# LANL-Bioinformatics/PCRamp

Measured on AMD Instinct MI355X. Metric: primer-pair x target amplification evals/sec, higher is better.
Workload: dtype u32

## Files before the change

### pcramp_amd/csrc/pcr_device.hip

```cpp
#include <hip/hip_runtime.h>
#include <cstring>
#include <rocprim/device/device_radix_sort.hpp>

#include <stdint.h>
#include <string.h>
#include <math.h>
#include <stdlib.h>
#include <string>
#include <vector>
#include <chrono>
#include <algorithm>
#include <unordered_map>
#include <type_traits>
#include <thread>
#include <mutex>
#include <condition_variable>
#include <functional>
#include <memory>
#include <atomic>
#include <cassert>
#include <sched.h>
#include <pthread.h>

#include "../../include/pcramp_hip.h"
// ... 464 lines not shown
		for(uint32_t j = k >> 1;j > 0;j >>= 1){
			for(uint32_t i = tid;i < np2;i += FINBIG_THREADS){
				const uint32_t l = i ^ j;
				if(l > i){
					const uint64_t a = fin_keys[i], b = fin_keys[l];
					const bool up = ((i & k) == 0);
					if((a > b) == up){ fin_keys[i] = b; fin_keys[l] = a; }
				}
			}
			__syncthreads();
		}
	}
	const uint32_t chunk = (np2 + FINBIG_THREADS - 1)/FINBIG_THREADS;
	const uint32_t lo = min(np2, tid*chunk), hi = min(np2, lo + chunk);
	uint32_t cnt = 0;
	for(uint32_t i = lo;i < hi;++i){
		const uint64_t k = fin_keys[i];
		if(k != ~0ull && (i == 0 || fin_keys[i - 1] != k)) ++cnt;
	}
	part[tid] = cnt;
	__syncthreads();
	if(tid == 0){
		uint32_t run = 0;
		for(int t = 0;t < FINBIG_THREADS;++t){ const uint32_t c = part[t]; part[t] = run; run += c; }
		seg_hi[seq] = seq*cap + run;
	}
	__syncthreads();
	uint32_t rank = part[tid];
	for(uint32_t i = lo;i < hi;++i){
		const uint64_t k = fin_keys[i];
		if(k != ~0ull && (i == 0 || fin_keys[i - 1] != k)){
			DevEntry e;
			materialise_entry(k, planes, blk_off, irr, irr_off, e);
			db[(size_t)seq*cap + rank] = e;
			++rank;
		}
	}
}

#include "pcr_screen.inc"

#include "pcr_sw.inc"
#include "pcr_thermo.inc"

constexpr uint32_t N_TOUCHED_UNKNOWN = 0xFFFFFFFFu;
constexpr uint32_t EPOCH_LIMIT = (1u << 24) - 1;

struct SeqSet {
	uint32_t n = 0;
	std::vector<std::vector<uint8_t> > packed;
	std::vector<uint64_t> len, blk_off, nblk_real;
	std::vector<float> weight; DevBuf<float> d_weight; bool weight_dirty = true;
	std::vector<uint8_t> active;
	std::vector<std::vector<pcrhost::IrrEntry> > irr_host;
	uint64_t total_blocks = 0;
	uint32_t n_tiles = 0, n_irr = 0;
	bool ctrl_clean = false;
	bool touched_from_seg = false;
	uint32_t bucket_cap = 64;
	DevBuf<uint32_t> irr_perm; uint32_t irr_size_count[256];
	DevBuf<uint4> planes;
	DevBuf<uint32_t> valid, nib, tb, blk_seq, tile_seq, tile_pos0, irr_off, degen_tiles;
	uint32_t *valid_d() const { return valid.p + S2_VALID_FRONT; }
	uint32_t *tb_d() const { return tb.p + S2_TB_FRONT; }
	DevBuf<uint8_t> tile_degen; uint32_t n_degen_tiles = 0;
	DevBuf<TileDesc> tile_desc;
	DevBuf<uint64_t> d_len, d_blk_off, d_nblk_real;
	DevBuf<uint8_t> d_active;
	std::vector<uint8_t> has_eos; DevBuf<uint8_t> d_has_eos;
	DevBuf<IrrDev> irr;
	DevBuf<IrrScan> irr_scan;
	DevBuf<uint32_t> irx_first, irx_last, irx_words, irx_sums; bool irx_valid = false, irx_usable = false;
	uint32_t irr_n_multi = 0;
	DevBuf<uint32_t> pix_first, pix_last, pix_sums, blk_info, blk_local, blk_tile0; DevBuf<uint4> pix_ent; std::vector<uint32_t> pix_start_h; uint64_t pix_generation = 0; bool pix_valid = false, pix_usable = false;
	DevBuf<uint8_t> codes; DevBuf<uint64_t> d_code_off; bool have_codes = false;
	bool have_db = false;
	uint32_t n_entries = 0;
	uint32_t db_cap = 0;
	uint64_t n_slots = 0;
	DevBuf<DevEntry> db;
	DevBuf<uint32_t> touched;
	DevBuf<uint32_t> ctrl;
	uint32_t n_touched = 0;
	bool touched_built = false;
	uint32_t *d_seg_hi = nullptr;
};

}

struct HostPool {
	std::vector<std::thread> th;
	std::mutex m; std::condition_variable cv_go, cv_done;
	std::function<void(unsigned)> fn; unsigned n_parts = 0, next = 0, pending = 0; uint64_t gen = 0; bool stop = false;
	explicit HostPool(unsigned n_workers){ for(unsigned i = 0;i < n_workers;++i) th.emplace_back([this]{ work(); }); }
	~HostPool(){ { std::lock_guard<std::mutex> lk(m); stop = true; } cv_go.notify_all(); for(std::thread &t : th) t.join(); }
	unsigned size() const { return (unsigned)th.size(); }
	void work()
	{
		uint64_t seen = 0;
		std::unique_lock<std::mutex> lk(m);
		while(true){
			cv_go.wait(lk, [&]{ return stop || gen != seen; });
			if(stop) return;
			seen = gen;
			while(next < n_parts){ const unsigned p = next++; lk.unlock(); fn(p); lk.lock(); }
			if(--pending == 0) cv_done.notify_one();
		}
	}
	void run(unsigned parts, std::function<void(unsigned)> f)
	{
		std::unique_lock<std::mutex> lk(m);
		fn = std::move(f); n_parts = parts; next = 0; pending = (unsigned)th.size(); ++gen;
		cv_go.notify_all();
		while(next < n_parts){ const unsigned p = next++; lk.unlock(); fn(p); lk.lock(); }
		cv_done.wait(lk, [&]{ return pending == 0; });
	}
};

namespace { struct PassJob; struct Launcher; }

struct ItemBufs {
	DevBuf<uint8_t> *tmp; DevBuf<uint32_t> *cnt; DevBuf<uint64_t> *eoff; DevBuf<uint2> *items;
	DevBuf<uint64_t> *joff; DevBuf<float4> *res; DevBuf<uint2> *item_tm; DevBuf<uint32_t> *flag;
};
struct ItemScratch {
	DevBuf<uint8_t> in, tmp; DevBuf<uint32_t> cnt, flag; DevBuf<uint64_t> eoff, joff, ioff; DevBuf<uint2> items, item_tm; DevBuf<float4> res;
	ItemBufs bufs() { return ItemBufs{&tmp, &cnt, &eoff, &items, &joff, &res, &item_tm, &flag}; }
};

struct pcr_ctx {
	int device = 0;
	std::unique_ptr<HostPool> pool_;
	HostPool &host_pool()
	{
		if(!pool_){ const unsigned hw = std::max(1u, std::thread::hardware_concurrency()); pool_.reset(new HostPool(std::min(hw, 16u) - 1u)); }
		return *pool_;
	}
	Stream stream;
	Stream aux_stream;
	std::string design_text;
	DevBuf<uint64_t> split_where;
	pcr_params params;
	pcrhost::PackFilter filt;
	SeqSet sets[PCR_N_SETS];
	DevBuf<uint32_t> best, counters, mask, status;
	int scan_version = 3;
	bool force_seed1 = false;
	pcrseed::Lister seed_lists;
	static constexpr int S3_CHUNK_SETS = pcrseed::CHUNK_SETS;
	struct S2Key { uint32_t a, c, g, t, floor_; bool operator==(const S2Key &o) const { return a == o.a && c == o.c && g == o.g && t == o.t && floor_ == o.floor_; } };
	struct S2KeyHash { size_t operator()(const S2Key &k) const { uint64_t h = 0x9E3779B97F4A7C15ull; for(uint32_t v : {k.a, k.c, k.g, k.t, k.floor_}){ h ^= v; h *= 0x100000001B3ull; h ^= h >> 29; } return (size_t)h; } };
	struct S2Entry { std::vector<uint32_t> seeds;  uint32_t off_mask; bool seedable; };
	std::vector<pcrhost::Seed> s2_tmp;
	struct S3Launch { Seed3Slices W; uint32_t n_chunks, per_wg, slice_cap, n_irr_wg; };
	int pair_mode = 1; bool s3_pair_attr_set = false;
	bool no_seed3 = false, s3_attr_set = false;
	bool s3_next = true;
	bool s2_attr_set = false; uint32_t s2_dbg = 0; bool no_irr_index = false;
	std::unordered_map<S2Key, S2Entry, S2KeyHash> s1_cache;
	DevBuf<uint32_t> s1_image, s1_heads, s1_multi, s1_part;
	bool host_seed_tables = false;
	DevBuf<Hit> hits;
	DevBuf<uint64_t> bits_fr, bits_rf;
	DevBuf<OligoDev> oligos;
	DevBuf<SwJob> sw_jobs; DevBuf<SwOut> sw_out; DevBuf<uint8_t> sw_q, sw_qlen, sw_t, entry_codes, entry_lens;
	DevBuf<AmpRec> amp_recs, amp_recs2; DevBuf<BgPairDev> bg_pairs;
	DevBuf<uint64_t> amp_keys; DevBuf<uint32_t> amp_pkeys, amp_pair_start; DevBuf<uint8_t> sort_tmp;
	DevBuf<thermo::Job> th_jobs; DevBuf<thermo::JobOut> th_out; DevBuf<int> th_dg; DevBuf<uint2> th_map; DevBuf<uint32_t> th_bad;
	float th_dg_salt = -1.0f;
	DevBuf<unsigned long long> th_dbg; bool th_attr_set = false;
	std::vector<thermo::Job> th_host_jobs; std::vector<thermo::JobOut> th_host_res;
	MappedBuf<uint8_t> sw_pin; Event sw_done[2];
	DevBuf<pcr_amplicon> mx_amp;
	DevBuf<OligoDev> opt_oligos; DevBuf<uint2> opt_jobs; DevBuf<float> opt_cov; DevBuf<uint32_t> opt_loc, opt_tasks;
	DevBuf<Planes> mx_keys; uint32_t mx_n_keys = 0; DevBuf<uint32_t> mx_count;
	DevBuf<uint8_t> pool_in, pool_tmp; DevBuf<uint32_t> pool_cnt, pool_ord; DevBuf<uint64_t> pool_eoff, pool_ioff, pool_keys; DevBuf<uint2> pool_items; DevBuf<pcr_product> pool_rec;
	DevBuf<uint8_t> site_in, site_tmp; DevBuf<uint32_t> site_cnt, site_ord, site_flag; DevBuf<uint64_t> site_eoff, site_joff, site_keys; DevBuf<uint2> site_items; DevBuf<float4> site_res; DevBuf<pcr_site> site_rec;
	bool site_attr_set = false;
	DevBuf<uint8_t> sv_item; DevBuf<uint32_t> sv_ord, sv_var, sv_start, sv_vord, sv_map; DevBuf<pcr_site_variant> sv_rec; DevBuf<uint64_t> sv_vkeys;
	bool sv_attr_set = false;
	DevBuf<uint4> rp_foot; DevBuf<uint64_t> rp_keys; DevBuf<uint32_t> rp_u32; DevBuf<uint8_t> rp_state; DevBuf<pcr_repair_step> rp_rec;
	pcr_comm *shard_comm = nullptr; uint64_t shard_first = 0, shard_n_total = 0; int shard_mode = 0;
	DevBuf<uint64_t> sh_rec, sh_full; DevBuf<uint8_t> sh_stage;
	std::vector<uint64_t> shard_bounds; DevBuf<uint64_t> d_shard_bounds;
	bool design_ready = false; DevBuf<uint64_t> sh_bits;
	std::vector<std::vector<uint8_t> > samp_packed; std::vector<uint64_t> samp_len;
	void drop_shard(){ shard_comm = nullptr; shard_mode = 0; shard_bounds.clear(); design_ready = false; samp_packed.clear(); samp_len.clear(); }
	pcr_comm *trial_comm = nullptr;
	size_t amp_cap = size_t(1) << 20;
	uint32_t n_cu = 256;
	DevBuf<uint64_t> fin_scratch;
	std::vector<uint16_t> seed_count; std::vector<uint8_t> seed_fill, seed_own;
	uint32_t epoch = 0;
	uint32_t debug_epoch = 0;
	bool opt_pm_global = false;
	uint32_t opt_dbg_wg_tasks = 0, opt_dbg_task_cap = 0;
	uint64_t best_seen = 0;
	static constexpr int STAGE_RING = 4;
	struct StageSlot { MappedBuf<uint8_t> buf; Event done; bool busy = false;
	                   uint32_t guard_seq = 0;  };
	StageSlot stage[STAGE_RING]; int stage_next = 0;
	struct DirectSlot { DevBuf<uint8_t> buf{true}; uint32_t guard_seq = 0; };
	DirectSlot dstage[STAGE_RING]; int dstage_next = 0;
	bool direct_ok = false;
	typedef PassMail Mail;
	static constexpr uint32_t MAIL_RING = 8;
	MappedBuf<Mail> mail;
	uint32_t mail_seq = 0;
	MappedBuf<uint8_t> ret;
	MappedBuf<uint8_t> in;
	MappedBuf<uint32_t> ret_flag; uint32_t ret_seq = 0;
	struct Pending {
		uint32_t seq; int which; std::vector<pcr_pair> pairs; int opt5, opt3; float thr; uint32_t min_len;
		pcr_amplify_args args; uint64_t *d_fr, *d_rf;
	};
	std::vector<Pending> pending;
	std::vector<std::vector<pcr_pair> > pair_pool;
	bool launch_thread = true;
	Launcher *launcher = nullptr; pcrq::Client lq_client; uint64_t n_pipelined = 0;
	std::mutex job_m; std::vector<PassJob *> job_free, job_all;
	DevBuf<uint8_t> arena;
	const uint4 *d_cand_fwd = nullptr, *d_cand_rc = nullptr; const uint32_t *d_cand_floor = nullptr;
	const OligoDev *d_oligos = nullptr;
	bool debug_log = false;
	bool timing = false; double t_host[8] = {0, 0, 0, 0, 0, 0, 0, 0}; uint64_t n_timed = 0;
	bool prof = false; uint32_t prof_stride = 1, prof_pass = 0;
	std::vector<std::pair<Event, Event> > prof_events;
	double prof_ms = 0.0; uint64_t prof_launches = 0;
	std::vector<std::pair<Event, Event> > prof_events_k[PCR_PROF_KERNELS];
	double prof_ms_k[PCR_PROF_KERNELS] = {0.0, 0.0, 0.0}; uint64_t prof_launches_k[PCR_PROF_KERNELS] = {0, 0, 0};
	DevBuf<uint8_t> pdim_in, pdim_tmp; DevBuf<float4> pdim_res; DevBuf<pcr_pool_dimer> pdim_rec, pdim_out; DevBuf<uint32_t> pdim_keep, pdim_off, pdim_flag;
	bool pdim_attr_set = false;
	DevBuf<uint32_t> ptm_ord; DevBuf<uint64_t> ptm_keys, ptm_bits; DevBuf<pcr_product_tm> ptm_rec;
	DevBuf<uint32_t> pph_hcnt, pph_ord; DevBuf<uint64_t> pph_hoff, pph_keys, pph_bits; DevBuf<uint4> pph_prod; DevBuf<pcr_probe_hit> pph_rec;
	DevBuf<uint4> pam_iv, pam_stat; DevBuf<uint32_t> pam_u32; DevBuf<uint64_t> pam_u64; DevBuf<pcr_amplicon_info> pam_info; DevBuf<uint8_t> pam_tmp, pam_packed;
	uint32_t bg_max_pairs = 0;
	uint32_t amp_dbg_hash_bits = 0;
	DevBuf<uint4> ppc_iv; DevBuf<uint32_t> ppc_pos, ppc_u32; DevBuf<uint64_t> ppc_u64; DevBuf<pcr_probe_candidate> ppc_rec; DevBuf<uint8_t> ppc_tmp;
	DevBuf<uint32_t> anp_pairseq; DevBuf<uint64_t> anp_out; DevBuf<float> anp_melt;
	DevBuf<uint8_t> pcf_din; DevBuf<uint32_t> pcf_vals, pcf_ucell, pcf_dkeep, pcf_keep, pcf_koff;
	DevBuf<uint64_t> pcf_aoff, pcf_keys; DevBuf<float4> pcf_dres;
	DevBuf<uint4> pcf_uagg, pcf_dense; DevBuf<pcr_pool_dimer> pcf_drec; DevBuf<float> pcf_dmat; DevBuf<pcr_pool_conflict> pcf_rec, pcf_out;
	ItemScratch shared;
	DevBuf<uint2> pe3_end; DevBuf<uint32_t> pe3_before, pe3_ord; DevBuf<uint64_t> pe3_sum, pe3_keys, pe3_bits; DevBuf<uint8_t> pe3_tmp;
	DevBuf<pcr_product_end3> pe3_rec;
	DevBuf<uint32_t> pde3_cnt, pde3_off, pde3_keep, pde3_koff; DevBuf<uint2> pde3_jobs; DevBuf<float4> pde3_res;
	DevBuf<pcr_pool_dimer_end3> pde3_rec, pde3_out; DevBuf<pcr_dimer_placement> pde3_place;
	bool pde3_attr_set = false;
	DevBuf<pcr_pool_dimer_end3> pcx_dense; DevBuf<pcr_pool_conflict_ext> pcx_rec, pcx_out;
};

namespace {

int drain(pcr_ctx *ctx);
int flush_launcher(pcr_ctx *ctx);
void detach_launcher(pcr_ctx *ctx);
void free_jobs(pcr_ctx *ctx);

struct ProfScope {
	pcr_ctx *ctx; int k; Event e0, e1;
	ProfScope(pcr_ctx *c, int kernel, bool on = true) : ctx(c), k(kernel)
	{
		if(!on || !ctx->prof || k < 0 || k >= PCR_PROF_KERNELS) return;
		if(e0.create() != hipSuccess || e1.create() != hipSuccess){ e0.release(); return; }
		(void)hipEventRecord(e0, ctx->stream);
	}
	void finish()
	{
		if(!e0) return;
		(void)hipEventRecord(e1, ctx->stream);
		((k == PCR_PROF_SCAN) ? ctx->prof_events : ctx->prof_events_k[k]).emplace_back(std::move(e0), std::move(e1));
	}
	~ProfScope() { finish(); }
};
constexpr int PCR_SET_SCRATCH = 3;
inline bool set_ok(pcr_set which) { return (unsigned)which <= (unsigned)PCR_SET_MULTIPLEX; }
#define CHECK_SET(which) do{ if(!set_ok(which)){ g_err = "unknown sequence set (PCR_SET_TARGET, PCR_SET_BACKGROUND or PCR_SET_MULTIPLEX)"; return PCR_ERR_ARG; } }while(0)
#define FLUSH(ctx) do{ if((ctx)->launcher){ const int frc_ = flush_launcher(ctx); if(frc_ != PCR_OK) return frc_; } }while(0)
#define DRAIN(ctx) do{ FLUSH(ctx); if(!(ctx)->pending.empty()){ const int drc_ = drain(ctx); if(drc_ != PCR_OK) return drc_; } }while(0)

struct HostTimer {
	pcr_ctx *ctx; int slot; std::chrono::steady_clock::time_point t0;
	HostTimer(pcr_ctx *c, int s) : ctx(c), slot(s) { if(ctx->timing) t0 = std::chrono::steady_clock::now(); }
	void next(int s)
	{
		if(!ctx->timing) return;
		const auto t1 = std::chrono::steady_clock::now();
		ctx->t_host[slot] += std::chrono::duration<double, std::micro>(t1 - t0).count();
		slot = s; t0 = t1;
	}
	~HostTimer() { next(slot); }
};

__global__ void k_apply_splits(const uint64_t *__restrict__ where, uint32_t n, uint32_t *__restrict__ planes , uint32_t *__restrict__ nib)
{
	const uint32_t i = blockIdx.x*blockDim.x + threadIdx.x;
	if(i >= n) return;
	const uint64_t gb = where[2*(size_t)i];
	const uint32_t bit = (uint32_t)where[2*(size_t)i + 1];
	const uint32_t m = ~(1u << bit);
	for(int k = 0;k < 4;++k) atomicAnd(&planes[gb*4 + k], m);
	atomicAnd(&nib[gb*4 + (bit >> 3)], ~(0xFu << ((bit & 7u)*4u)));
}

int upload_irregular(pcr_ctx *ctx, SeqSet &S)
{
	const auto tu0 = std::chrono::steady_clock::now();
	auto ms_since = [&](){ return std::chrono::duration<double, std::milli>(std::chrono::steady_clock::now() - tu0).count(); };
	double t_flat = 0, t_sort = 0, t_scan = 0, t_copy1 = 0;
	size_t total = 0;
	for(uint32_t s = 0;s < S.n;++s) total += S.irr_host[s].size();
	std::vector<IrrDev> flat(total);
	std::vector<uint32_t> off(S.n + 1, 0);
	for(int k = 0;k < 256;++k) S.irr_size_count[k] = 0;
	{
		size_t at = 0;
		for(uint32_t s = 0;s < S.n;++s){
			off[s] = (uint32_t)at;
			const std::vector<pcrhost::IrrEntry> &v = S.irr_host[s];
			for(size_t k = 0;k < v.size();++k){
				const pcrhost::IrrEntry &e = v[k];
				IrrDev &d = flat[at++];
				d.w = e.w; d.loc = e.loc; d.seq = s;
				d.meta = (uint32_t)e.strand | ((uint32_t)e.cws << 8) | ((uint32_t)e.ord << 16);
				d.local_id = (uint32_t)k;
				++S.irr_size_count[e.cws & 0xFF];
			}
		}
	}
	off[S.n] = (uint32_t)flat.size();
	S.n_irr = (uint32_t)flat.size();
	t_flat = ms_since();
	std::vector<uint32_t> perm(flat.size());
	t_sort = ms_since();
	int rc;
	{
		auto spread = [](uint64_t v) -> uint64_t {
			v = (v | (v << 16)) & 0x0000FFFF0000FFFFull; v = (v | (v << 8)) & 0x00FF00FF00FF00FFull; v = (v | (v << 4)) & 0x0F0F0F0F0F0F0F0Full;
			v = (v | (v << 2)) & 0x3333333333333333ull; v = (v | (v << 1)) & 0x5555555555555555ull; return v;
		};
		uint32_t start[256];
		uint32_t run = 0;
		for(int k = 255;k >= 0;--k){ start[k] = run; run += S.irr_size_count[k]; }
		std::vector<IrrScan> scan(perm.size());
		uint32_t n_multi = 0;
		for(size_t i = 0;i < flat.size();++i){
			const IrrDev &d = flat[i];
			const uint32_t at = start[(d.meta >> 8) & 0xFF]++;
			perm[at] = (uint32_t)i;
			const uint32_t multi = (d.w.a & d.w.c) | (d.w.a & d.w.g) | (d.w.a & d.w.t) | (d.w.c & d.w.g) | (d.w.c & d.w.t) | (d.w.g & d.w.t);
			if(multi) ++n_multi;
			const uint32_t lo = d.w.c | d.w.t, hi = d.w.g | d.w.t;
			const uint64_t code = spread(lo) | (spread(hi) << 1);
			IrrScan r; r.w0 = (uint32_t)code; r.w1 = (uint32_t)(code >> 32); r.idx_flags = (uint32_t)i | (multi ? 0x80000000u : 0u); r.seq = d.seq;
			scan[at] = r;
		}
		S.irr_n_multi = n_multi; S.irx_valid = false;
		t_scan = ms_since();
		if((rc = S.irr_scan.ensure_slack(scan.size() + 1)) != PCR_OK) return rc;
		if(!scan.empty()) HIP_TRY(hipMemcpy(S.irr_scan.p, scan.data(), scan.size()*sizeof(IrrScan), hipMemcpyHostToDevice));
	}
	t_copy1 = ms_since();
	if((rc = S.irr_perm.ensure_slack(perm.size() + 1)) != PCR_OK) return rc;
	if(!perm.empty()) HIP_TRY(hipMemcpyAsync(S.irr_perm.p, perm.data(), perm.size()*sizeof(uint32_t), hipMemcpyHostToDevice, ctx->stream));
	if((rc = S.irr.ensure_slack(flat.size())) != PCR_OK) return rc;
	if((rc = S.irr_off.ensure(off.size())) != PCR_OK) return rc;
	if(!flat.empty()) HIP_TRY(hipMemcpyAsync(S.irr.p, flat.data(), flat.size()*sizeof(IrrDev), hipMemcpyHostToDevice, ctx->stream));
	HIP_TRY(hipMemcpyAsync(S.irr_off.p, off.data(), off.size()*sizeof(uint32_t), hipMemcpyHostToDevice, ctx->stream));
	HIP_TRY(hipStreamSynchronize(ctx->stream));
	if(ctx->timing && flat.size() > 100000) fprintf(stderr, "[pcramp] irregular list of %zu words: flat %.1f  order %.1f  scan records %.1f  first copy %.1f  other copies %.1f ms\n", flat.size(), t_flat, t_sort - t_flat, t_scan - t_sort, t_copy1 - t_scan, ms_since() - t_copy1);
	return PCR_OK;
}

void launch_exclusive_scan(pcr_ctx *ctx, uint32_t *counts, uint32_t *starts, uint32_t n, uint32_t *sums)
{
	const uint32_t n_blocks = (n + 4095u)/4096u;
	hipLaunchKernelGGL(k_scan_blocks, dim3(n_blocks), dim3(1024), 0, ctx->stream, counts, starts, n, sums);
	hipLaunchKernelGGL(k_scan_sums, dim3(1), dim3(1024), 0, ctx->stream, sums, n_blocks);
	hipLaunchKernelGGL(k_scan_add, dim3(n_blocks), dim3(1024), 0, ctx->stream, starts, counts, n, sums);
}

constexpr uint32_t IRX_MAX_RUN = 1024;
int ensure_irr_index(pcr_ctx *ctx, SeqSet &S)
{
	if(S.irx_valid) return PCR_OK;
	int rc;
	if((rc = S.irx_first.ensure(IRX_KEYS + 4)) != PCR_OK) return rc;
	if((rc = S.irx_last.ensure(IRX_KEYS + 4)) != PCR_OK) return rc;
	if((rc = S.irx_words.ensure_slack((size_t)24*S.n_irr + 4)) != PCR_OK) return rc;
	const uint32_t n_blocks = (IRX_KEYS + 4095u)/4096u;
	if((rc = S.irx_sums.ensure(n_blocks + 4)) != PCR_OK) return rc;
	HIP_TRY(hipMemsetAsync(S.irx_last.p, 0, (size_t)IRX_KEYS*sizeof(uint32_t), ctx->stream));
	if(S.n_irr){
		hipLaunchKernelGGL(k_irx_count, dim3((S.n_irr + 255)/256), dim3(256), 0, ctx->stream, S.irr.p, S.n_irr, S.irx_last.p);
		HIP_TRY(hipGetLastError());
	}
	{
		uint32_t longest = 0;
		HIP_TRY(hipMemsetAsync(S.irx_sums.p + n_blocks, 0, sizeof(uint32_t), ctx->stream));
		hipLaunchKernelGGL(k_irx_max, dim3(256), dim3(256), 0, ctx->stream, S.irx_last.p, IRX_KEYS, S.irx_sums.p + n_blocks);
		HIP_TRY(hipMemcpyAsync(&longest, S.irx_sums.p + n_blocks, sizeof(uint32_t), hipMemcpyDeviceToHost, ctx->stream));
		HIP_TRY(hipStreamSynchronize(ctx->stream));
// ... 297 lines not shown
	HIP_TRY(hipMemcpyAsync(&n, S.ctrl.p + 3, sizeof(uint32_t), hipMemcpyDeviceToHost, ctx->stream));
	HIP_TRY(hipStreamSynchronize(ctx->stream));
	S.n_touched = n; S.n_entries = n ? 1 : 0; S.touched_built = true;
	return PCR_OK;
}

int amplify_launch(pcr_ctx *ctx, SeqSet &S, const pcr_pair *pairs, uint32_t n_pairs, const pcr_amplify_args *a,
	uint64_t *d_fr, uint64_t *d_rf, const FusedAmp *fa = nullptr)
{
	{ const int erc = ensure_touched(ctx, S); if(erc != PCR_OK) return erc; }
	if(!S.have_db){ g_err = "pcr_amplify: no word DB (call pcr_select_words first)"; return PCR_ERR_STATE; }
	const uint64_t words = (S.n + 63)/64;
	const size_t bits_bytes = (size_t)n_pairs*words*sizeof(uint64_t);
	if(S.n_entries == 0 || n_pairs == 0){
		if(bits_bytes){
			HIP_TRY(hipMemsetAsync(d_fr, 0, bits_bytes, ctx->stream));
			HIP_TRY(hipMemsetAsync(d_rf, 0, bits_bytes, ctx->stream));
		}
		return PCR_OK;
	}
	HostTimer timer(ctx, 4);
	int rc;
	const bool prestaged = fa && fa->staged;
	if(prestaged) ctx->d_oligos = fa->d_oligos;
	else{
		std::vector<OligoDev> ol;
		build_oligos(pairs, n_pairs, a, ol);
		Stager st(ctx);
		if((rc = st.begin(ol.size()*sizeof(OligoDev) + 64)) != PCR_OK) return rc;
		ctx->d_oligos = st.put(ol.data(), ol.size());
		const bool vec_ok = ((uintptr_t)d_fr % 16 == 0) && ((uintptr_t)d_rf % 16 == 0) && (bits_bytes % 16 == 0);
		if(!vec_ok){
			HIP_TRY(hipMemsetAsync(d_fr, 0, bits_bytes, ctx->stream));
			HIP_TRY(hipMemsetAsync(d_rf, 0, bits_bytes, ctx->stream));
		}
		if((rc = vec_ok ? st.ship(d_fr, bits_bytes, d_rf, bits_bytes) : st.ship()) != PCR_OK) return rc;
	}
	timer.next(5);
	const uint32_t mask_words = (2*n_pairs + 31)/32;
	if((rc = ctx->mask.ensure((size_t)S.n_slots*mask_words)) != PCR_OK) return rc;
	if((rc = ctx->status.ensure(1)) != PCR_OK) return rc;
	const bool dev_n = S.n_touched == N_TOUCHED_UNKNOWN;
	const uint32_t *n_dev = dev_n ? S.ctrl.p + 3 : nullptr;
	const uint32_t n_t = dev_n ? 0u : S.n_touched, n_db = n_t*S.db_cap;
	const unsigned threads = dev_n ? 256 : 128;
	const unsigned grid = dev_n ? (unsigned)std::min<uint64_t>(((uint64_t)S.n*S.db_cap + threads - 1)/threads, 1024) : (n_db + threads - 1)/threads;
	const unsigned mgrid = dev_n ? std::min<unsigned>((S.n + MATCH_WAVES - 1)/MATCH_WAVES, 1024u) : (n_t + MATCH_WAVES - 1)/MATCH_WAVES;
	hipLaunchKernelGGL(k_match, dim3(std::max(mgrid, 1u)), dim3(64*MATCH_WAVES), 0, ctx->stream, S.db.p, n_t, n_dev, S.db_cap,
		S.touched.p, S.d_seg_hi, ctx->d_oligos, 2*n_pairs, mask_words, ctx->mask.p, ctx->status.p,
		prestaged ? fa->pub_counters : (const uint32_t *)nullptr, prestaged ? ctx->mail.dev + (fa->pub_seq % pcr_ctx::MAIL_RING) : (pcr_ctx::Mail *)nullptr,
		prestaged ? fa->pub_seq : 0u);
	HIP_TRY(hipGetLastError());
	hipLaunchKernelGGL(k_pair, dim3(grid), dim3(threads), 0, ctx->stream, S.db.p, n_db, n_dev, S.db_cap, S.touched.p, S.d_seg_hi, ctx->mask.p,
		mask_words, ctx->d_oligos, n_pairs, S.planes.p, S.d_blk_off.p, S.d_len.p, S.d_active.p, a->amp_min, a->amp_max,
		a->ident_threshold, a->use_taq_mama, d_fr, d_rf, words, ctx->status.p);
	HIP_TRY(hipGetLastError());
	return PCR_OK;
}

template<int NSLOT, int KLO>
int launch_scan2_nw(pcr_ctx *ctx, SeqSet &S, uint32_t nw, uint32_t group0, uint32_t n_groups, uint32_t gw, uint32_t ncand, const HitSink &sink,
	const uint32_t *d_tab, const uint32_t *d_bias, const uint32_t *tile_ids, uint32_t n_tiles, const uint32_t *orient_ids)
{
#define SCAN2_ARGS S.nib.p, S.planes.p, S.valid_d(), S.d_blk_off.p, S.d_len.p, S.d_active.p, S.tile_seq.p, S.tile_pos0.p, \
	d_tab, d_bias, group0, gw, tile_ids, orient_ids, ctx->d_cand_fwd, ctx->d_cand_rc, ctx->d_cand_floor, ncand, sink
	const dim3 grid(n_tiles, n_groups), block(SCAN2_THREADS);
	switch(nw){
		case 1: hipLaunchKernelGGL((k_scan2<1, NSLOT, KLO>), grid, block, 0, ctx->stream, SCAN2_ARGS); break;
		case 2: hipLaunchKernelGGL((k_scan2<2, NSLOT, KLO>), grid, block, 0, ctx->stream, SCAN2_ARGS); break;
		case 3: hipLaunchKernelGGL((k_scan2<3, NSLOT, KLO>), grid, block, 0, ctx->stream, SCAN2_ARGS); break;
		case 4: hipLaunchKernelGGL((k_scan2<4, NSLOT, KLO>), grid, block, 0, ctx->stream, SCAN2_ARGS); break;
		case 5: hipLaunchKernelGGL((k_scan2<5, NSLOT, KLO>), grid, block, 0, ctx->stream, SCAN2_ARGS); break;
		case 6: hipLaunchKernelGGL((k_scan2<6, NSLOT, KLO>), grid, block, 0, ctx->stream, SCAN2_ARGS); break;
		case 7: hipLaunchKernelGGL((k_scan2<7, NSLOT, KLO>), grid, block, 0, ctx->stream, SCAN2_ARGS); break;
		default: hipLaunchKernelGGL((k_scan2<8, NSLOT, KLO>), grid, block, 0, ctx->stream, SCAN2_ARGS); break;
	}
#undef SCAN2_ARGS
	HIP_TRY(hipGetLastError());
	return PCR_OK;
}

int launch_scan2(pcr_ctx *ctx, SeqSet &S, const Scan2Tables &T, uint32_t ncand, const HitSink &sink,
	const uint32_t *d_tab, const uint32_t *d_bias, const uint32_t *tile_ids, uint32_t n_tiles, const uint32_t *orient_ids)
{
	if(n_tiles == 0 || T.n_groups == 0) return PCR_OK;
	const uint32_t full = (T.last_words == T.gw) ? T.n_groups : T.n_groups - 1;
	int rc = PCR_OK;
	if(full){
		rc = (T.nslot == 26) ? launch_scan2_nw<26, 3>(ctx, S, T.gw, 0, full, T.gw, ncand, sink, d_tab, d_bias, tile_ids, n_tiles, orient_ids)
			: launch_scan2_nw<32, 0>(ctx, S, T.gw, 0, full, T.gw, ncand, sink, d_tab, d_bias, tile_ids, n_tiles, orient_ids);
		if(rc != PCR_OK) return rc;
	}
	if(full < T.n_groups){
		rc = (T.nslot == 26) ? launch_scan2_nw<26, 3>(ctx, S, T.last_words, full, 1, T.gw, ncand, sink, d_tab, d_bias, tile_ids, n_tiles, orient_ids)
			: launch_scan2_nw<32, 0>(ctx, S, T.last_words, full, 1, T.gw, ncand, sink, d_tab, d_bias, tile_ids, n_tiles, orient_ids);
	}
	return rc;
}

int count_entries(pcr_ctx *ctx, SeqSet &S)
{
	uint64_t total = 0;
	if(S.n_touched){
		std::vector<uint32_t> hi(S.n);
		HIP_TRY(hipMemcpyAsync(hi.data(), S.d_seg_hi, S.n*sizeof(uint32_t), hipMemcpyDeviceToHost, ctx->stream));
		HIP_TRY(hipStreamSynchronize(ctx->stream));
		for(uint32_t q = 0;q < S.n;++q){ if(hi[q]) total += hi[q] - (uint64_t)q*S.db_cap; }
	}
	S.n_entries = (uint32_t)total;
	return PCR_OK;
}

}

extern "C" {

const char *pcr_last_error(void) { return g_err.c_str(); }

pcr_ctx *pcr_create(int device, void *hip_stream, const pcr_params *params)
{
	int count = 0;
	if(hipGetDeviceCount(&count) != hipSuccess || count <= 0){
		g_err = "pcr_create: no HIP device available (this library has no CPU fallback)";
		return nullptr;
	}
	if(device < 0 || device >= count){ g_err = "pcr_create: bad device index"; return nullptr; }
	if(hipSetDevice(device) != hipSuccess){ g_err = "pcr_create: hipSetDevice failed"; return nullptr; }
	hipDeviceProp_t prop;
	if(hipGetDeviceProperties(&prop, device) != hipSuccess){ g_err = "pcr_create: hipGetDeviceProperties failed"; return nullptr; }
	if(std::string(prop.gcnArchName).find("gfx950") == std::string::npos){
		g_err = std::string("pcr_create: device is ") + prop.gcnArchName + ", this build targets gfx950 only";
		return nullptr;
	}
	pcr_ctx *ctx = new pcr_ctx();
	ctx->device = device;
	if(hip_stream) ctx->stream.borrow((hipStream_t)hip_stream);
	else if(ctx->stream.create() != hipSuccess){ g_err = "pcr_create: hipStreamCreate failed"; delete ctx; return nullptr; }
	if(params){ ctx->params = *params; }
	else{ ctx->params.pack_max_degen = 256; ctx->params.pack_min_gc = 0.0f; ctx->params.pack_max_gc = 1.0f; }
	{ hipDeviceProp_t prop; if(hipGetDeviceProperties(&prop, device) == hipSuccess && prop.multiProcessorCount > 0) ctx->n_cu = (uint32_t)prop.multiProcessorCount; }
	if(const char *v = getenv("PCRAMP_TIMING")) ctx->timing = v[0] == '1';
	ctx->debug_log = getenv("PCRAMP_DEBUG") != nullptr;
	if(const char *v = getenv("PCRAMP_DEBUG_EPOCH")) ctx->debug_epoch = (uint32_t)strtoul(v, nullptr, 0);
	if(const char *v = getenv("PCRAMP_OPT_PM")) ctx->opt_pm_global = v[0] == 'g';
	if(const char *v = getenv("PCRAMP_DEBUG_OPT_TASKS")){ unsigned a = 0, b = 0; if(sscanf(v, "%u,%u", &a, &b) >= 1){ ctx->opt_dbg_wg_tasks = a; ctx->opt_dbg_task_cap = b; } }
	if(const char *v = getenv("PCRAMP_DEBUG_AMP_HASH_BITS")) ctx->amp_dbg_hash_bits = (uint32_t)strtoul(v, nullptr, 0);
	if(const char *v = getenv("PCRAMP_DEBUG_AMP_CAP")) ctx->amp_cap = std::max<size_t>(16, (size_t)strtoull(v, nullptr, 0));
	if(const char *v = getenv("PCRAMP_SEED")) ctx->force_seed1 = v[0] == '1';
	if(const char *v = getenv("PCRAMP_SEED_TABLES")) ctx->host_seed_tables = v[0] == 'h';
	if(const char *v = getenv("PCRAMP_S2DBG")) ctx->s2_dbg = (uint32_t)atoi(v);
	if(const char *v = getenv("PCRAMP_IRR_INDEX")) ctx->no_irr_index = v[0] == '0';
	if(const char *v = getenv("PCRAMP_SEED3")) ctx->no_seed3 = v[0] == '0';
	if(const char *v = getenv("PCRAMP_S3_NEXT")) ctx->s3_next = v[0] != '0';
	if(const char *v = getenv("PCRAMP_SEED_MEMO")) ctx->seed_lists.use_memo = v[0] != '0';
	if(const char *v = getenv("PCRAMP_LAUNCH_THREAD")) ctx->launch_thread = v[0] != '0';
	if(const char *v = getenv("PCRAMP_PAIR")) ctx->pair_mode = (v[0] == '0') ? 0 : (strcmp(v, "force") == 0) ? 2 : 1;
	if(const char *v = getenv("PCRAMP_SCAN")){ if(v[0] == '1') ctx->scan_version = 1; else if(v[0] == '2') ctx->scan_version = 2; }
	{
		const char *v = getenv("PCRAMP_STAGE");
		if(!(v && v[0] == 'k') && prop.isLargeBar){
			DevBuf<uint32_t> probe(true); MappedBuf<uint32_t> back; const std::string err_before = g_err;
			constexpr uint32_t PROBE_WORDS = 1024;
			if(probe.ensure(PROBE_WORDS) == PCR_OK && back.ensure(PROBE_WORDS*sizeof(uint32_t)) == PCR_OK){
				hipPointerAttribute_t at;
				bool ok = hipPointerGetAttributes(&at, probe.p) == hipSuccess;
				for(int round = 0;ok && round < 2;++round){
					volatile uint32_t *w = (volatile uint32_t *)probe.p;
					for(uint32_t i = 0;i < PROBE_WORDS;++i){ w[i] = 0x9E3779B9u*(i + 1) + (uint32_t)round; back.host[i] = 0; }
					__builtin_ia32_sfence();
					hipLaunchKernelGGL(k_stage, dim3(1), dim3(256), 0, ctx->stream, (const uint4 *)probe.p, (uint4 *)back.dev, PROBE_WORDS/4,
						(uint4 *)nullptr, 0u, (uint4 *)nullptr, 0u, (uint4 *)nullptr, 0u);
					ok = hipGetLastError() == hipSuccess && hipStreamSynchronize(ctx->stream) == hipSuccess;
					for(uint32_t i = 0;ok && i < PROBE_WORDS;++i) ok = back.host[i] == 0x9E3779B9u*(i + 1) + (uint32_t)round;
				}
				ctx->direct_ok = ok;
			}
			else{ (void)hipGetLastError(); g_err = err_before; }
		}
	}
	ctx->filt.max_degen = ctx->params.pack_max_degen;
	ctx->filt.set_gc(ctx->params.pack_min_gc, ctx->params.pack_max_gc);
	if(hipMemcpyToSymbol(HIP_SYMBOL(c_taq_mama), h_taq_mama, sizeof(h_taq_mama)) != hipSuccess ||
	   hipMemcpyToSymbol(HIP_SYMBOL(thermo::c_H), PCR_NN_H, sizeof(PCR_NN_H)) != hipSuccess ||
	   hipMemcpyToSymbol(HIP_SYMBOL(thermo::c_S), PCR_NN_S, sizeof(PCR_NN_S)) != hipSuccess ||
	   hipMemcpyToSymbol(HIP_SYMBOL(thermo::c_loop_S), PCR_LOOP_S, sizeof(PCR_LOOP_S)) != hipSuccess ||
	   hipMemcpyToSymbol(HIP_SYMBOL(thermo::c_bulge_S), PCR_BULGE_S, sizeof(PCR_BULGE_S)) != hipSuccess ||
	   hipMemcpyToSymbol(HIP_SYMBOL(thermo::c_hairpin_S), PCR_HAIRPIN_S, sizeof(PCR_HAIRPIN_S)) != hipSuccess ||
	   hipMemcpyToSymbol(HIP_SYMBOL(thermo::c_special_H), PCR_SPECIAL_H, sizeof(PCR_SPECIAL_H)) != hipSuccess ||
	   hipMemcpyToSymbol(HIP_SYMBOL(thermo::c_special_S), PCR_SPECIAL_S, sizeof(PCR_SPECIAL_S)) != hipSuccess ||
	   hipMemcpyToSymbol(HIP_SYMBOL(thermo::c_special_key), PCR_SPECIAL_KEY, sizeof(PCR_SPECIAL_KEY)) != hipSuccess ||
	   hipMemcpyToSymbol(HIP_SYMBOL(thermo::c_wc), PCR_WC, sizeof(PCR_WC)) != hipSuccess){
		g_err = "pcr_create: hipMemcpyToSymbol failed"; delete ctx; return nullptr;
	}
	if(ctx->mail.ensure(sizeof(pcr_ctx::Mail)*pcr_ctx::MAIL_RING) != PCR_OK){ g_err = "pcr_create: mapped host allocation failed"; delete ctx; return nullptr; }
	memset((void *)ctx->mail.host, 0, sizeof(pcr_ctx::Mail)*pcr_ctx::MAIL_RING);
	return ctx;
}

void pcr_destroy(pcr_ctx *ctx)
{
	if(!ctx) return;
	(void)hipSetDevice(ctx->device);
	(void)flush_launcher(ctx);
	detach_launcher(ctx);
	(void)hipStreamSynchronize(ctx->stream);
	if(ctx->aux_stream) (void)hipStreamSynchronize(ctx->aux_stream);
	ctx->pending.clear();
	free_jobs(ctx);
	if(ctx->timing && ctx->n_timed){
		const double n = (double)ctx->n_timed;
		fprintf(stderr, "[pcramp] host us/pass by stage: A (plan, caller's thread) %.1f  B (stage + launch, %s) %.1f  (%llu of %llu passes pipelined, queue depth <= %u)\n",
			ctx->t_host[0]/n, ctx->n_pipelined ? "launcher thread" : "caller's thread", (ctx->t_host[1] + ctx->t_host[2])/n,
			(unsigned long long)ctx->n_pipelined, (unsigned long long)ctx->n_timed, ctx->lq_client.max_depth);
		fprintf(stderr, "[pcramp] host us/pass: plan %.1f  stage %.1f  launch %.1f  wait %.1f | amplify prep %.1f  launch %.1f  (%llu passes)\n",
			ctx->t_host[0]/n, ctx->t_host[1]/n, ctx->t_host[2]/n, ctx->t_host[3]/n, ctx->t_host[4]/n, ctx->t_host[5]/n, (unsigned long long)ctx->n_timed);
	}
	delete ctx;
}

uint32_t pcr_num_sequences(pcr_ctx *ctx, pcr_set which) { return (ctx && set_ok(which)) ? ctx->sets[which].n : 0; }
uint64_t pcr_bitset_words(pcr_ctx *ctx, pcr_set which) { return (ctx && set_ok(which)) ? (ctx->sets[which].n + 63)/64 : 0; }

int pcr_staging_mode(pcr_ctx *ctx) { return (ctx && ctx->direct_ok) ? 1 : 0; }

int pcr_launcher_stats(pcr_ctx *ctx, uint64_t *passes_pipelined, uint32_t *max_queue_depth)
{
	if(!ctx){ g_err = "null ctx"; return PCR_ERR_ARG; }
	if(passes_pipelined) *passes_pipelined = ctx->n_pipelined;
	if(max_queue_depth) *max_queue_depth = ctx->lq_client.max_depth;
	return PCR_OK;
}

int pcr_live_resources(uint64_t out[4])
{
	if(!out){ g_err = "pcr_live_resources: bad argument"; return PCR_ERR_ARG; }
	for(int k = 0;k < 4;++k) out[k] = pcrown::g_live[k].load();
	return PCR_OK;
}

int pcr_synchronize(pcr_ctx *ctx)
{
	if(!ctx){ g_err = "null ctx"; return PCR_ERR_ARG; }
	HIP_TRY(hipSetDevice(ctx->device));
	DRAIN(ctx);
	HIP_TRY(hipStreamSynchronize(ctx->stream));
	return PCR_OK;
}

static int load_sequences_impl(pcr_ctx *ctx, int which, const uint8_t *packed4, const uint64_t *byte_offsets,
	const uint64_t *lengths, const float *weights, uint32_t n);

int pcr_load_sequences(pcr_ctx *ctx, pcr_set which, const uint8_t *packed4, const uint64_t *byte_offsets,
	const uint64_t *lengths, const float *weights, uint32_t n)
{
	if(!set_ok(which)){ g_err = "pcr_load_sequences: unknown sequence set"; return PCR_ERR_ARG; }
	return load_sequences_impl(ctx, (int)which, packed4, byte_offsets, lengths, weights, n);
}

static int load_sequences_impl(pcr_ctx *ctx, int which, const uint8_t *packed4, const uint64_t *byte_offsets,
	const uint64_t *lengths, const float *weights, uint32_t n)
{
	if(!ctx || which < 0 || which >= PCR_N_SETS || (n && (!packed4 || !byte_offsets || !lengths))){
		g_err = "pcr_load_sequences: bad argument"; return PCR_ERR_ARG;
	}
	DRAIN(ctx);
	if(n >= (1u << 24)){ g_err = "pcr_load_sequences: at most 2^24-1 sequences per GPU shard"; return PCR_ERR_CAPACITY; }
	HIP_TRY(hipSetDevice(ctx->device));
	HIP_TRY(hipStreamSynchronize(ctx->stream));
	SeqSet &S = ctx->sets[which];
	S.have_db = false; S.n_entries = 0; S.have_codes = false;
	S.n = n;
	S.packed.assign(n, std::vector<uint8_t>());
	S.len.assign(lengths, lengths + n);
	if(which == PCR_SET_TARGET) ctx->drop_shard();
	if(which == PCR_SET_TARGET || which == PCR_SET_BACKGROUND) ctx->trial_comm = nullptr;
	S.weight.assign(n, 1.0f);
	if(weights) S.weight.assign(weights, weights + n);
	S.weight_dirty = true;
	S.ctrl_clean = false; S.touched_from_seg = false;
	S.active.assign(n, 1);
	S.has_eos.assign(n, 0);
	S.blk_off.assign(n + 1, 0);
	S.nblk_real.assign(n, 0);
	S.irr_host.assign(n, std::vector<pcrhost::IrrEntry>());
	uint64_t total_bytes = 0, total_blocks = 0, n_tiles = 0;
	std::vector<uint64_t> dev_byte_off(n);
	for(uint32_t s = 0;s < n;++s){
		if(lengths[s] >= (uint64_t(1) << 31)){ g_err = "pcr_load_sequences: sequence longer than 2^31-1 bases"; return PCR_ERR_CAPACITY; }
		const uint64_t nb = (lengths[s] + 1)/2;
		S.packed[s].assign(packed4 + byte_offsets[s], packed4 + byte_offsets[s] + nb);
		if((lengths[s] & 1) && nb) S.packed[s][nb - 1] &= 0xF0;
		{
			const std::vector<uint8_t> &b = S.packed[s];
			bool eos = false;
			const uint64_t full = lengths[s]/2;
			for(uint64_t k = 0;k < full && !eos;++k) eos = ((b[k] & 0xF0) == 0) || ((b[k] & 0x0F) == 0);
			if(!eos && (lengths[s] & 1)) eos = ((b[full] & 0xF0) == 0);
			S.has_eos[s] = eos ? 1 : 0;
		}
		dev_byte_off[s] = total_bytes;
		total_bytes += nb;
		S.blk_off[s] = total_blocks;
		S.nblk_real[s] = (lengths[s] + 31)/32;
		total_blocks += S.nblk_real[s] + 2;
		if(lengths[s] >= 32) n_tiles += (lengths[s] - 7 + TILE_POS - 1)/TILE_POS;
	}
// ... 508 lines not shown
```

### pcramp_amd/csrc/pcr_scan_seed3.inc

```

constexpr uint32_t PIX_CODES = 1u << 18;
constexpr uint32_t PIX_KEYS = PIX_CODES << 2;
constexpr uint32_t S3_BATCH = 8;

template<bool SCATTER>
__global__ void k_pix_build(const uint32_t *__restrict__ tb, const uint32_t *__restrict__ blk_seq, const uint64_t *__restrict__ blk_off,
	const uint64_t *__restrict__ len, uint64_t total_blocks, uint32_t *__restrict__ count_or_cursor, uint4 *__restrict__ ent)
{
	const uint64_t b = (uint64_t)blockIdx.x*blockDim.x + threadIdx.x;
	if(b >= total_blocks) return;
	const uint32_t seq = blk_seq[b];
	const int64_t p0 = (int64_t)(b - blk_off[seq])*32, L = (int64_t)len[seq];
	uint32_t w[8];
#pragma unroll
	for(int k = 0;k < 8;++k) w[k] = tb[(int64_t)2*(int64_t)b - 2 + k];
#pragma unroll
	for(int i = 0;i < 32;++i){
		if(p0 + i + 9 > L) break;
		const uint32_t ten = (i < 16) ? funnel(w[2], w[3], 2*i) : funnel(w[3], w[4], 2*(i - 16));
		const uint32_t code = ((ten & S2_CODE_MASK) << 2) | ((ten >> 18) & 3u);
		if(SCATTER){
			const uint32_t at = atomicAdd(&count_or_cursor[code], 1u);
			const int jl = (i + 9) >> 4, sl = 2*((i + 9) & 15);
			const int jr = (i + 41) >> 4, sr = 2*((i + 41) & 15);
			const uint32_t l_lo = funnel(w[jl], w[jl + 1], sl), l_hi = funnel(w[jl + 1], w[jl + 2], sl) & 0x3FFFu;
			const uint32_t r_lo = funnel(w[jr], w[jr + 1], sr), r_hi = funnel(w[jr + 1], w[jr + 2], sr) & 0x3FFFu;
			ent[at] = make_uint4((uint32_t)(b*32 + (uint64_t)i), l_lo, l_hi | (r_lo << 14), (r_lo >> 18) | (r_hi << 14));
		}
		else atomicAdd(&count_or_cursor[code], 1u);
	}
}

struct Seed3Tables {
	const uint32_t *seeds;
	const uint32_t *chunk_prefix;
	const uint8_t *spans;
	const uint4 *masks; const uint8_t *floors;
	uint32_t n_seeds, n_or, or_base;
	const uint32_t *pix_first, *pix_last; const uint4 *pix_ent;
	uint32_t n_chunks, per_wg, slice_cap;
	uint32_t n_irr_wg;
};
constexpr uint32_t S3_MAX_WG = 512;
constexpr uint32_t S3_MAX_OR = 448, S3_MAX_SEEDS = 1u << 16;
struct Seed3Slices { uint32_t start[S3_MAX_WG + 1]; };
struct Seed3Set {
	const uint32_t *valid, *blk_info, *blk_local; const uint8_t *active;
};
constexpr uint32_t BLK_SEQ_MASK = 0x3FFFFFFFu, BLK_INACTIVE = 0x40000000u, BLK_DEGEN = 0x80000000u;

__global__ void k_blk_info(const uint32_t *__restrict__ blk_seq, const uint64_t *__restrict__ blk_off, const uint64_t *__restrict__ len,
	const uint32_t *__restrict__ tile0, const uint8_t *__restrict__ tile_degen, const uint8_t *__restrict__ active, uint64_t total_blocks,
	uint32_t *__restrict__ blk_info, uint32_t *__restrict__ blk_local)
{
	const uint64_t b = (uint64_t)blockIdx.x*blockDim.x + threadIdx.x;
	if(b >= total_blocks) return;
	const uint32_t q = blk_seq[b];
	const uint64_t bl = b - blk_off[q], tile = bl >> 5;
	const uint32_t nt = tile0[q + 1] - tile0[q];
	const bool degen = tile < nt && tile_degen[tile0[q] + tile];
	blk_info[b] = q | (degen ? 0x80000000u : 0u) | (active[q] ? 0u : 0x40000000u);
	blk_local[b] = (uint32_t)bl;
}

__global__ void k_blk_active(uint32_t *__restrict__ blk_info, const uint32_t *__restrict__ blk_seq, const uint8_t *__restrict__ active, uint64_t total_blocks)
{
	const uint64_t b = (uint64_t)blockIdx.x*blockDim.x + threadIdx.x;
	if(b >= total_blocks) return;
	const uint32_t v = blk_info[b] & ~BLK_INACTIVE;
	blk_info[b] = v | (active[blk_seq[b]] ? 0u : BLK_INACTIVE);
}

__device__ __forceinline__ void s3_irregular(const Seed3Tables &T3, const Seed3Set &Q, const IrrArgs2 &IA, const uint4 *__restrict__ cand_fwd,
	const uint32_t *__restrict__ cand_floor, HitSink sink, uint32_t gw, uint32_t n_gw, uint32_t lane)
{
	for(uint32_t i0 = gw*16u;i0 < T3.n_seeds;i0 += n_gw*16u){
		const uint32_t i = i0 + lane;
		const uint32_t sdv = (lane < 16u && i < T3.n_seeds) ? T3.seeds[i] : S2_END;
		const uint32_t orient = T3.or_base + (sdv & 0x1FFu);
		uint32_t first = 0, cnt = 0;
		if(sdv != S2_END && !(orient & 1u)){
			const uint32_t key = (((sdv >> 9) & 31u) << 18) | (sdv >> 14);
			first = IA.ix_first[key]; cnt = IA.ix_last[key] - first;
		}
		const uint32_t incl = s2_scan(cnt);
		const uint32_t total = s2_rl(incl, 63);
		for(uint32_t t0 = 0;t0 < total;t0 += 64u){
			const uint32_t t = t0 + lane;
			uint32_t lo = 0;
#pragma unroll
			for(uint32_t stp = 32u;stp;stp >>= 1){ if((uint32_t)__shfl((int)incl, (int)(lo + stp - 1u)) <= t) lo += stp; }
			const int sl = (int)min(lo, 63u);
			const uint32_t s_incl = (uint32_t)__shfl((int)incl, sl), s_cnt = (uint32_t)__shfl((int)cnt, sl), s_first = (uint32_t)__shfl((int)first, sl);
			const uint32_t c = (uint32_t)__shfl((int)orient, sl) >> 1;
			if(t >= total) continue;
			const IrrDev e = IA.irr[IA.ix_words[s_first + (t - (s_incl - s_cnt))]];
			if(((e.meta >> 8) & 0xFFu) < IA.min_cws || !Q.active[e.seq]) continue;
			const uint32_t n = match_count(e.w.a, e.w.c, e.w.g, e.w.t, cand_fwd[c]);
			if(n >= cand_floor[c]) record_hit(sink, e.seq, c, make_key(e.seq, e.loc, e.meta & 0xFF, 1, (e.meta >> 16) & 0xFF), n);
		}
	}
}

template<uint32_t S3_THREADS>
__global__ __launch_bounds__(S3_THREADS) __attribute__((amdgpu_waves_per_eu(8, 8))) void k_seed3(Seed3Tables T3, Seed3Set Q, IrrArgs2 IA, const uint4 *__restrict__ cand_fwd, const uint32_t *__restrict__ cand_floor,
	HitSink sink, S2Clear Z, Seed3Slices W)
{
#include "pcr_scan_seed3_pass.inc"
}

struct Seed3Row {
	Seed3Tables T3; Seed3Set Q; IrrArgs2 IA; const uint4 *cand_fwd; const uint32_t *cand_floor; HitSink sink; S2Clear Z;
};
struct Seed3HalfSlices { uint32_t start[S3_MAX_WG/2 + 1]; };
template<uint32_t S3_THREADS>
__global__ __launch_bounds__(S3_THREADS) __attribute__((amdgpu_waves_per_eu(8, 8))) void k_seed3_pair(Seed3Row A, Seed3HalfSlices WA, Seed3Row B, Seed3HalfSlices WB)
{
	if(blockIdx.y == 0){
		const Seed3Tables &T3 = A.T3; const Seed3Set &Q = A.Q; const IrrArgs2 &IA = A.IA; const uint4 *const cand_fwd = A.cand_fwd; const uint32_t *const cand_floor = A.cand_floor;
		const HitSink &sink = A.sink; const S2Clear &Z = A.Z; const Seed3HalfSlices &W = WA;
#include "pcr_scan_seed3_pass.inc"
	}
	else{
		const Seed3Tables &T3 = B.T3; const Seed3Set &Q = B.Q; const IrrArgs2 &IA = B.IA; const uint4 *const cand_fwd = B.cand_fwd; const uint32_t *const cand_floor = B.cand_floor;
		const HitSink &sink = B.sink; const S2Clear &Z = B.Z; const Seed3HalfSlices &W = WB;
#include "pcr_scan_seed3_pass.inc"
	}
}
```

### pcramp_amd/csrc/pcr_scan_seed3_pass.inc

```
	extern __shared__ uint4 s3_dyn[];
	uint4 *const masks = s3_dyn;
	uint32_t *const prefix = (uint32_t *)(masks + T3.n_or);
	uint32_t *const seeds = prefix + T3.slice_cap;
	uint8_t *const floors = (uint8_t *)(seeds + T3.slice_cap);
	uint8_t *const spans = floors + ((T3.n_or + 15u) & ~15u);
	const uint32_t wave = (uint32_t)__builtin_amdgcn_readfirstlane((int)(threadIdx.x >> 6)), lane = threadIdx.x & 63u;
	for(uint32_t i = blockIdx.x*S3_THREADS + threadIdx.x;i < Z.n0;i += gridDim.x*S3_THREADS) Z.z0[i] = make_uint4(0, 0, 0, 0);
	for(uint32_t i = blockIdx.x*S3_THREADS + threadIdx.x;i < Z.n1;i += gridDim.x*S3_THREADS) Z.z1[i] = make_uint4(0, 0, 0, 0);
	if(Z.ctrl && blockIdx.x == 0 && threadIdx.x == 0){ Z.ctrl[1] = 0; Z.ctrl[3] = 0; }
	for(uint32_t i = threadIdx.x;i < T3.n_or;i += S3_THREADS){ masks[i] = T3.masks[i]; floors[i] = T3.floors[i]; }
	constexpr uint32_t S3_WAVES = S3_THREADS/64;
	if(blockIdx.x < T3.n_irr_wg){
		if(IA.ix_first) s3_irregular(T3, Q, IA, cand_fwd, cand_floor, sink, blockIdx.x*S3_WAVES + wave, T3.n_irr_wg*S3_WAVES, lane);
		return;
	}
	const uint32_t wg = blockIdx.x - T3.n_irr_wg, n_wg = gridDim.x - T3.n_irr_wg;
	const uint32_t s_lo = W.start[wg];
	const uint32_t n_slice = min(min(W.start[wg + 1] + 2u, T3.n_seeds + 1u) - s_lo, T3.slice_cap);
	for(uint32_t i = threadIdx.x;i < n_slice;i += S3_THREADS){ prefix[i] = T3.chunk_prefix[s_lo + i]; const bool in = s_lo + i < T3.n_seeds; seeds[i] = in ? T3.seeds[s_lo + i] : 0u; spans[i] = in ? T3.spans[s_lo + i] : (uint8_t)0; }
	__syncthreads();
	const uint32_t gw = wg*S3_WAVES + wave, n_gw = n_wg*S3_WAVES;
	const uint32_t q_lo = wg*T3.per_wg, q_hi = min(q_lo + T3.per_wg, T3.n_chunks);
	for(uint32_t q0 = q_lo + wave;q0 < q_hi;q0 += S3_WAVES*S3_BATCH){
		uint32_t c_first = 0, c_cnt = 0, c_sd = 0;
		{
			const uint32_t q = q0 + lane*S3_WAVES;
			if(lane < S3_BATCH && q < q_hi){
				uint32_t lo = 0, hi = n_slice - 1u;
				while(hi - lo > 1u){ const uint32_t mid = (lo + hi) >> 1; if(prefix[mid] <= q) lo = mid; else hi = mid; }
				c_sd = seeds[lo];
				const uint32_t key = (c_sd >> 14) << 2, sp = spans[lo];
				const uint32_t f = T3.pix_first[key + (sp & 3u)], e = T3.pix_last[key + (sp >> 2)], j0 = (q - prefix[lo])*64u;
				c_first = f + j0; c_cnt = (e - f) - j0;
			}
		}
		uint4 en[S3_BATCH];
#pragma unroll
		for(int b = 0;b < (int)S3_BATCH;++b){
			const uint32_t first = s2_rl(c_first, b), cnt = s2_rl(c_cnt, b);
			en[b] = make_uint4(0xFFFFFFFFu, 0, 0, 0);
			if(lane < cnt) en[b] = T3.pix_ent[first + lane];
		}
		uint32_t cnt_b[S3_BATCH], g[S3_BATCH]; bool pass_b[S3_BATCH];
#pragma unroll
		for(int b = 0;b < (int)S3_BATCH;++b){
			const uint32_t sdv = s2_rl(c_sd, b);
			const uint32_t off = (sdv >> 9) & 31u, local = sdv & 0x1FFu, code = sdv >> 14;
			g[b] = en[b].x;
			const uint32_t r_lo = funnel(en[b].z, en[b].w, 14);
			const uint4 cx = make_uint4(en[b].y << 2, (funnel(en[b].y, en[b].z, 30) & 0xFFFFu) | (code << 16), (code >> 16) | (r_lo << 2), en[b].w >> 12);
			const uint32_t in = 24u - off, sh = 2u*(in & 15u);
			const uint32_t a0 = (in < 16u) ? funnel(cx.x, cx.y, sh) : funnel(cx.y, cx.z, sh);
			const uint32_t a1 = (in < 16u) ? funnel(cx.y, cx.z, sh) : funnel(cx.z, cx.w, sh);
			cnt_b[b] = (uint32_t)__popc(s2_mux(a0, a1, masks[local]));
			pass_b[b] = g[b] != 0xFFFFFFFFu && cnt_b[b] >= floors[local] && g[b] >= off;
		}
		uint32_t vw[S3_BATCH], info[S3_BATCH], bl[S3_BATCH];
#pragma unroll
		for(int b = 0;b < (int)S3_BATCH;++b){
			vw[b] = 0; info[b] = 0; bl[b] = 0;
			if(pass_b[b]){
				const uint32_t ws = g[b] - ((s2_rl(c_sd, b) >> 9) & 31u);
				vw[b] = Q.valid[ws >> 5]; info[b] = Q.blk_info[ws >> 5]; bl[b] = Q.blk_local[ws >> 5];
			}
		}
#pragma unroll
		for(int b = 0;b < (int)S3_BATCH;++b){
			if(!pass_b[b]) continue;
			const uint32_t sdv = s2_rl(c_sd, b);
			const uint32_t ws = g[b] - ((sdv >> 9) & 31u), seq = info[b] & BLK_SEQ_MASK;
			if(!((vw[b] >> (ws & 31u)) & 1u) || (info[b] & (BLK_DEGEN | BLK_INACTIVE))) continue;
			const uint32_t p_local = bl[b]*32u + (ws & 31u);
			const uint32_t orient = T3.or_base + (sdv & 0x1FFu), c = orient >> 1;
			if(orient & 1u) record_hit(sink, seq, c, make_key(seq, (int32_t)p_local + 31, 2, 0, 0), cnt_b[b]);
			else record_hit(sink, seq, c, make_key(seq, (int32_t)p_local, 1, 0, 0), cnt_b[b]);
		}
	}
	if(IA.ix_first && T3.n_irr_wg == 0) s3_irregular(T3, Q, IA, cand_fwd, cand_floor, sink, gw, n_gw, lane);
```

### pcramp_amd/csrc/pcr_seed_lists.hpp

```cpp
#ifndef PCR_SEED_LISTS_HPP
#define PCR_SEED_LISTS_HPP

#include <stddef.h>
#include <stdint.h>
#include <stdlib.h>
#include <string.h>
#include <new>
#include <unordered_map>
#include <vector>
#include "pcr_host.hpp"

namespace pcrseed {

using pcrhost::Planes;

struct Mask16 { uint32_t x, y, z, w; };

inline uint32_t spread16(uint32_t v)
{
	v &= 0xFFFFu;
	v = (v | (v << 8)) & 0x00FF00FFu; v = (v | (v << 4)) & 0x0F0F0F0Fu;
	v = (v | (v << 2)) & 0x33333333u; return (v | (v << 1)) & 0x55555555u;
}
inline Mask16 mask_of(const Planes &m)
{
	const Mask16 r = { spread16(m.a) | (spread16(m.a >> 16) << 1), spread16(m.c) | (spread16(m.c >> 16) << 1),
	                   spread16(m.g) | (spread16(m.g >> 16) << 1), spread16(m.t) | (spread16(m.t >> 16) << 1) };
	return r;
}

template<class T> struct RawBuf {
	T *p = nullptr; size_t n = 0, cap = 0;
	RawBuf() {}
	RawBuf(const RawBuf &) = delete; RawBuf &operator=(const RawBuf &) = delete;
	~RawBuf() { free(p); }
	T *data() { return p; } const T *data() const { return p; }
	size_t size() const { return n; } bool empty() const { return n == 0; }
	T &operator[](size_t i) { return p[i]; } const T &operator[](size_t i) const { return p[i]; }
	void clear() { n = 0; }
	void resize(size_t want)
	{
		if(want > cap){
			const size_t c = want + want/2 + 64;
			T *q = (T *)realloc(p, c*sizeof(T));
			if(!q) throw std::bad_alloc();
			p = q; cap = c;
		}
		n = want;
	}
};

struct Key { uint32_t a, c, g, t, floor_; bool operator==(const Key &o) const { return a == o.a && c == o.c && g == o.g && t == o.t && floor_ == o.floor_; } };
struct KeyHash { size_t operator()(const Key &k) const { uint64_t h = 0x9E3779B97F4A7C15ull; for(uint32_t v : {k.a, k.c, k.g, k.t, k.floor_}){ h ^= v; h *= 0x100000001B3ull; h ^= h >> 29; } return (size_t)h; } };

constexpr int CHUNK_SETS = 4;

struct EntryHead {
	Mask16 mask = {0, 0, 0, 0}; uint32_t off_mask = 0, n = 0; bool seedable = false;
	uint32_t next_slot = 0, total[CHUNK_SETS] = {0, 0, 0, 0}; uint64_t gen[CHUNK_SETS] = {0, 0, 0, 0};
	uint32_t *block = nullptr;
};
struct Entry : EntryHead {
	Entry() {}
	Entry(Entry &&o) : EntryHead(o) { o.block = nullptr; }
	Entry(const Entry &) = delete; Entry &operator=(const Entry &) = delete;
	~Entry() { free(block); }
	const uint32_t *seeds() const { return block; }
	uint32_t *run(int slot) const { return block + (size_t)(1 + slot)*n; }
	const uint8_t *spans() const { return (const uint8_t *)(block + (size_t)(1 + CHUNK_SETS)*n); }
	void alloc(uint32_t n_seeds, bool third)
	{
		n = n_seeds;
		const size_t bytes = third ? (size_t)(1 + CHUNK_SETS)*n*sizeof(uint32_t) + n : (size_t)n*sizeof(uint32_t);
		block = (uint32_t *)malloc(bytes ? bytes : 1);
		if(!block) throw std::bad_alloc();
	}
};

struct Cache {
	struct Slot { Key key; Entry *e; };
	std::unordered_map<Key, Entry, KeyHash> map;
	std::vector<Slot> memo;
	void clear() { map.clear(); memo.clear(); }
};

struct SetIndex { const uint32_t *start; uint64_t generation; };

struct Limits { uint32_t max_or, max_seeds; size_t lds_fixed, lds_budget; uint32_t max_groups; };

struct Lister {
	Cache second, third;
	size_t clear_above = 16384;
	bool use_memo = true;
	std::vector<pcrhost::Seed> tmp; std::vector<pcrhost::FoldSeed> tmp3;
	struct Rec { const Entry *e; const uint32_t *run; uint32_t tag, pf_base; };
	std::vector<Rec> recs; std::vector<uint32_t> rec_end, g_total;
};

struct SeedLists {
	RawBuf<uint32_t> s2_seeds; RawBuf<Mask16> s2_masks;
	std::vector<uint32_t> s2_group_end, s2_group_offmask, s2_group_or, s2_group_nor;
	RawBuf<uint32_t> s3_prefix;
	RawBuf<uint8_t> s3_spans;
};

inline Entry *derive(Lister &Z, Cache &C, const Key &key, const Planes &m, bool third, bool fold)
{
	Entry e;
	Z.tmp.clear();
	if(third){
		Z.tmp3.clear();
		e.seedable = pcrhost::orientation_index_seeds(m, key.floor_, fold, Z.tmp3, Z.tmp);
		e.alloc((uint32_t)Z.tmp3.size(), true);
		uint8_t *sp = (uint8_t *)e.spans();
		for(size_t k = 0;k < Z.tmp3.size();++k){
			const pcrhost::FoldSeed &sd = Z.tmp3[k];
			e.block[k] = (sd.code << 14) | ((uint32_t)sd.off << 9); sp[k] = (uint8_t)(sd.lo | (sd.hi << 2)); e.off_mask |= 1u << sd.off;
		}
	}
	else{
		e.seedable = pcrhost::orientation_seeds(m, key.floor_, 0, Z.tmp, nullptr, 9);
		e.alloc((uint32_t)Z.tmp.size(), false);
		for(size_t k = 0;k < Z.tmp.size();++k){ const pcrhost::Seed &sd = Z.tmp[k]; e.block[k] = (sd.code << 14) | ((uint32_t)sd.off << 9); e.off_mask |= 1u << sd.off; }
	}
	e.mask = mask_of(m);
	return &C.map.emplace(key, std::move(e)).first->second;
}

inline int chunk_slot(Entry &e, const SetIndex &S)
{
	for(int s = 0;s < CHUNK_SETS;++s){ if(e.gen[s] == S.generation) return s; }
	const int s = (int)e.next_slot; e.next_slot = (e.next_slot + 1u) % CHUNK_SETS;
	const uint32_t *const sd = e.seeds(); const uint8_t *const sp = e.spans(); uint32_t *const out = e.run(s);
	uint32_t run = 0;
	for(uint32_t k = 0;k < e.n;++k){
		const uint32_t key4 = (sd[k] >> 14) << 2, span = sp[k];
		out[k] = run; run += (S.start[key4 + (span >> 2) + 1u] - S.start[key4 + (span & 3u)] + 63u) >> 6;
	}
	e.total[s] = run; e.gen[s] = S.generation;
	return s;
}

inline bool list_seeds(Lister &Z, const Limits &lim, const pcrhost::Candidate *cand, size_t n_cand, const SetIndex *S3, bool fold,
	SeedLists &L, std::vector<uint32_t> &or_seed, std::vector<uint32_t> &or_plain, uint32_t &irr_off_mask)
{
	const uint32_t n_or = 2*(uint32_t)n_cand;
	const bool third = S3 != nullptr;
	L.s2_seeds.clear(); L.s3_prefix.clear(); L.s3_spans.clear();
	L.s2_group_end.clear(); L.s2_group_offmask.clear(); L.s2_group_or.clear(); L.s2_group_nor.clear();
	irr_off_mask = 0;
	L.s2_masks.resize(n_or);
	if(Z.second.map.size() > Z.clear_above) Z.second.clear();
	if(Z.third.map.size() > Z.clear_above) Z.third.clear();
	Cache &C = third ? Z.third : Z.second;
	if(Z.use_memo && C.memo.size() < n_or) C.memo.resize(n_or, Cache::Slot{Key{0, 0, 0, 0, 0}, nullptr});
	auto fits = [&lim](size_t n, uint32_t g_or){ return g_or <= lim.max_or && n <= lim.max_seeds && lim.lds_fixed + 17*(size_t)g_or + 8*n <= lim.lds_budget; };
	Z.recs.clear(); Z.rec_end.clear(); Z.g_total.clear();
	size_t n_out = 0, group_begin = 0; uint32_t group_mask = 0, group_or0 = 0, group_last = 0, pf_run = 0;
	Mask16 *const masks = L.s2_masks.data();
	for(uint32_t o = 0;o < n_or;++o){
		const pcrhost::Candidate &c = cand[o >> 1];
		const Planes &m = (o & 1u) ? c.rc : c.fwd;
		const Key key = {m.a, m.c, m.g, m.t, c.floor_};
		Entry *e;
		Cache::Slot *const memo = Z.use_memo ? &C.memo[o] : nullptr;
		if(memo && memo->e && memo->key == key) e = memo->e;
		else{
			auto it = C.map.find(key);
			e = it != C.map.end() ? &it->second : derive(Z, C, key, m, third, fold);
			if(memo){ memo->key = key; memo->e = e; }
		}
		masks[o] = e->mask;
		if(!e->seedable){ or_plain.push_back(o); continue; }
		or_seed.push_back(o);
		if(!fits(n_out - group_begin + e->n, o - group_or0 + 1)){
			if(!fits(e->n, 1) || L.s2_group_end.size() + 1 >= lim.max_groups) return false;
			L.s2_group_end.push_back((uint32_t)n_out); L.s2_group_offmask.push_back(group_mask); L.s2_group_or.push_back(group_or0); L.s2_group_nor.push_back(group_last - group_or0 + 1);
			Z.rec_end.push_back((uint32_t)Z.recs.size()); Z.g_total.push_back(pf_run);
			group_begin = n_out; group_mask = 0; group_or0 = o; pf_run = 0;
		}
		group_last = o;
		Lister::Rec r = { e, nullptr, o - group_or0, pf_run };
		if(third){ const int s = chunk_slot(*e, *S3); r.run = e->run(s); pf_run += e->total[s]; }
		Z.recs.push_back(r);
		n_out += e->n;
		if(!(o & 1u)){ irr_off_mask |= e->off_mask; group_mask |= e->off_mask; }
	}
	L.s2_group_end.push_back((uint32_t)n_out); L.s2_group_offmask.push_back(group_mask); L.s2_group_or.push_back(group_or0);
	L.s2_group_nor.push_back(or_seed.empty() ? 0u : group_last - group_or0 + 1);
	Z.rec_end.push_back((uint32_t)Z.recs.size()); Z.g_total.push_back(pf_run);
	L.s2_seeds.resize(n_out);
	if(third){ L.s3_spans.resize(n_out); L.s3_prefix.resize(n_out + Z.rec_end.size()); }
	uint32_t *__restrict out = L.s2_seeds.data(), *__restrict pf = L.s3_prefix.data(); uint8_t *__restrict spans = L.s3_spans.data();
	size_t r0 = 0;
	for(size_t g = 0;g < Z.rec_end.size();++g){
		for(size_t i = r0;i < Z.rec_end[g];++i){
			const Lister::Rec &r = Z.recs[i];
			const uint32_t n = r.e->n, tag = r.tag;
			const uint32_t *__restrict sd = r.e->seeds();
			for(uint32_t k = 0;k < n;++k) out[k] = sd[k] | tag;
			out += n;
			if(third){
				const uint32_t *__restrict run = r.run; const uint32_t base = r.pf_base;
				for(uint32_t k = 0;k < n;++k) pf[k] = base + run[k];
				pf += n;
				if(n){ memcpy(spans, r.e->spans(), n); spans += n; }
			}
		}
		r0 = Z.rec_end[g];
		if(third) *pf++ = Z.g_total[g];
	}
	return true;
}

template<class Launch>
inline bool plan_slices(const SeedLists &PL, std::vector<Launch> &launch, uint32_t G_all, uint32_t seeds_per_turn, uint32_t max_wg, size_t lds_budget, bool with_irr)
{
	launch.resize(PL.s2_group_end.size());
	size_t g_begin = 0, g_prefix = 0;
	for(size_t g = 0;g < PL.s2_group_end.size();++g){
		const uint32_t ns = PL.s2_group_end[g] - (uint32_t)g_begin;
		g_begin = PL.s2_group_end[g];
		const uint32_t *P = PL.s3_prefix.data() + g_prefix;
		g_prefix += (size_t)ns + 1;
		Launch &L = launch[g];
		L.n_irr_wg = with_irr ? std::min<uint32_t>((ns + seeds_per_turn - 1u)/seeds_per_turn, G_all/4u) : 0u;
		const uint32_t G = (G_all - L.n_irr_wg) & ~1u;
		L.n_chunks = P[ns]; L.per_wg = std::max<uint32_t>(1u, (L.n_chunks + G - 1u)/G); L.slice_cap = 2;
		if(ns == 0) continue;
		uint32_t at = 0;
		for(uint32_t w = 0;w <= G;++w){
			const uint64_t target = (uint64_t)w*L.per_wg;
			while(at + 1u < ns && P[at + 1u] <= target) ++at;
			L.W.start[w] = at;
		}
		for(uint32_t w = G + 1;w <= max_wg;++w) L.W.start[w] = at;
		for(uint32_t w = 0;w < G;++w) L.slice_cap = std::max(L.slice_cap, std::min(L.W.start[w + 1] + 2u, ns + 1u) - L.W.start[w]);
		if(17*(size_t)PL.s2_group_nor[g] + 9*(size_t)L.slice_cap + 64 > lds_budget) return false;
	}
	return true;
}

}

#endif
```

### pcramp_amd/csrc/pcr_select.inc

```
namespace {

struct PlanLists : pcrseed::SeedLists {
	std::vector<uint8_t> s2_floors;
	std::vector<pcr_ctx::S3Launch> s3_launch;
	std::vector<uint32_t> s1_seeds;
	void clear()
	{
		s2_seeds.clear(); s2_masks.clear(); s2_floors.clear(); s2_group_end.clear(); s2_group_offmask.clear(); s2_group_or.clear(); s2_group_nor.clear();
		s3_launch.clear(); s3_prefix.clear(); s3_spans.clear(); s1_seeds.clear();
	}
};

constexpr uint32_t S2_MAX_GROUPS = 4096;
static_assert(sizeof(pcrseed::Mask16) == sizeof(uint4) && alignof(pcrseed::Mask16) <= alignof(uint4), "the mask entry is the device's uint4");
static_assert(offsetof(pcrseed::Mask16, y) == offsetof(uint4, y) && offsetof(pcrseed::Mask16, w) == offsetof(uint4, w), "the mask entry is the device's uint4");
static_assert(S2_Q == 9, "pcrseed::derive lists 9-gram seeds");
static_assert(pcrseed::CHUNK_SETS == pcr_ctx::S3_CHUNK_SETS, "generations kept per cache entry");
bool plan_seed2(pcr_ctx *ctx, PlanLists &L, const std::vector<pcrhost::Candidate> &cand, std::vector<uint32_t> &or_seed, std::vector<uint32_t> &or_plain, uint32_t &irr_off_mask,
	const SeqSet *S3 = nullptr)
{
	const pcrseed::Limits lim2 = { S2_MAX_OR, S2_MAX_SEEDS, sizeof(S2Shared) + 1024, 160*1024, S2_MAX_GROUPS };
	const pcrseed::Limits lim3 = { S3_MAX_OR, S3_MAX_SEEDS, 0, ~size_t(0), S2_MAX_GROUPS };
	pcrseed::SetIndex ix = { nullptr, 0 };
	if(S3){ ix.start = S3->pix_start_h.data(); ix.generation = S3->pix_generation; }
	return pcrseed::list_seeds(ctx->seed_lists, S3 ? lim3 : lim2, cand.data(), cand.size(), S3 ? &ix : nullptr, ctx->s3_next, L, or_seed, or_plain, irr_off_mask);
}

constexpr size_t S3_LDS_BUDGET = 120*1024;
constexpr uint32_t S3_WG_THREADS = 1024;
uint32_t seed3_grid(const pcr_ctx *ctx) { return std::min<uint32_t>(2*ctx->n_cu, S3_MAX_WG); }
bool plan_seed3_slices(pcr_ctx *ctx, PlanLists &PL, bool with_irr)
{
	return pcrseed::plan_slices(PL, PL.s3_launch, seed3_grid(ctx), 16u*(S3_WG_THREADS/64), S3_MAX_WG, S3_LDS_BUDGET, with_irr);
}

void plan_seed1(pcr_ctx *ctx, PlanLists &L, const std::vector<pcrhost::Candidate> &cand, std::vector<uint32_t> &or_seed, std::vector<uint32_t> &or_plain, uint32_t &irr_off_mask)
{
	const uint32_t n_or = 2*(uint32_t)cand.size();
	std::vector<uint32_t> &out = L.s1_seeds;
	out.clear();
	irr_off_mask = 0;
	if(ctx->s1_cache.size() > 16384) ctx->s1_cache.clear();
	std::vector<const pcr_ctx::S2Entry *> ent(n_or);
	size_t total = 0;
	for(uint32_t o = 0;o < n_or;++o){
		const pcrhost::Candidate &c = cand[o >> 1];
		const Planes &m = (o & 1u) ? c.rc : c.fwd;
		const pcr_ctx::S2Key key = {m.a, m.c, m.g, m.t, c.floor_};
		auto it = ctx->s1_cache.find(key);
		if(it == ctx->s1_cache.end()){
			pcr_ctx::S2Entry e; e.off_mask = 0;
			ctx->s2_tmp.clear();
			e.seedable = pcrhost::orientation_seeds(m, c.floor_, 0, ctx->s2_tmp);
			e.seeds.reserve(ctx->s2_tmp.size());
			for(const pcrhost::Seed &sd : ctx->s2_tmp){ e.seeds.push_back(sd.code | ((uint32_t)sd.off << 16)); e.off_mask |= 1u << sd.off; }
			it = ctx->s1_cache.emplace(key, std::move(e)).first;
		}
		ent[o] = &it->second;
		if(ent[o]->seedable) total += ent[o]->seeds.size();
	}
	std::vector<uint8_t> drop(n_or, 0);
	if(total > S1_MAX_SEEDS){
		std::vector<uint32_t> by_len;
		for(uint32_t o = 0;o < n_or;++o){ if(ent[o]->seedable) by_len.push_back(o); }
		std::stable_sort(by_len.begin(), by_len.end(), [&](uint32_t x, uint32_t y){ return ent[x]->seeds.size() > ent[y]->seeds.size(); });
		for(size_t i = 0;i < by_len.size() && total > S1_MAX_SEEDS;++i){ drop[by_len[i]] = 1; total -= ent[by_len[i]]->seeds.size(); }
	}
	out.resize(total);
	size_t at = 0;
	for(uint32_t o = 0;o < n_or;++o){
		const pcr_ctx::S2Entry &e = *ent[o];
		if(!e.seedable || drop[o]){ or_plain.push_back(o); continue; }
		or_seed.push_back(o);
		const uint32_t tag = o << 21;
		for(size_t k = 0;k < e.seeds.size();++k) out[at + k] = e.seeds[k] | tag;
		at += e.seeds.size();
		if(!(o & 1u)) irr_off_mask |= e.off_mask;
	}
}

struct HostSeedPlan {
	std::vector<pcrhost::Seed> seeds;
	std::vector<std::vector<std::pair<uint16_t, int8_t> > > inheritors;
	size_t n_inherited = 0;
	std::vector<uint32_t> image, heads, multi;
};

int plan_seed_host(pcr_ctx *ctx, const std::vector<pcrhost::Candidate> &cand, HostSeedPlan &H, std::vector<uint32_t> &or_seed, std::vector<uint32_t> &or_plain,
	uint32_t &irr_off_mask)
{
	const uint32_t n_or = 2*(uint32_t)cand.size();
	struct OrientInfo { uint32_t begin, end; int max_exact_pos; bool seeded; };
	std::vector<OrientInfo> info;
	std::vector<pcrhost::Seed> &seeds = H.seeds;
	std::vector<std::vector<std::pair<uint16_t, int8_t> > > &inheritors = H.inheritors;
	size_t &n_inherited = H.n_inherited;
	std::vector<uint32_t> &image = H.image, &heads = H.heads, &multi = H.multi;
	info.assign(n_or, OrientInfo());
	inheritors.assign(n_or, std::vector<std::pair<uint16_t, int8_t> >());
	seeds.reserve((size_t)n_or*32);
	for(uint32_t o = 0;o < n_or;++o){
		const pcrhost::Candidate &c = cand[o >> 1];
		OrientInfo &me = info[o];
		me.begin = (uint32_t)seeds.size(); me.max_exact_pos = -1;
		const uint32_t bo = 2*c.base + (o & 1u);
		const int32_t sh = (o & 1u) ? -c.shift : c.shift;
		if(c.base != (o >> 1) && info[bo].seeded && info[bo].max_exact_pos <= 24 && info[bo].max_exact_pos + sh <= 24){
			inheritors[bo].push_back(std::make_pair((uint16_t)o, (int8_t)sh));
			n_inherited += info[bo].end - info[bo].begin;
			me.seeded = true; me.max_exact_pos = (info[bo].max_exact_pos < 0) ? -1 : info[bo].max_exact_pos + sh;
		}
		else me.seeded = pcrhost::orientation_seeds((o & 1) ? c.rc : c.fwd, c.floor_, o, seeds, &me.max_exact_pos);
		me.end = (uint32_t)seeds.size();
		if(me.seeded) or_seed.push_back(o); else or_plain.push_back(o);
	}
	if(or_seed.empty()) return PCR_OK;
	if(ctx->seed_count.size() != 65536){ ctx->seed_count.assign(65536, 0); ctx->seed_own.assign(65536, 0); }
	std::vector<uint16_t> &count = ctx->seed_count;
	bool overflow = false;
	uint32_t distinct = 0;
	std::vector<uint8_t> &own = ctx->seed_own;
	for(;;){
		image.assign(SEED_IMAGE_WORDS, 0u);
		overflow = false; distinct = 0;
		for(const pcrhost::Seed &sd : seeds){
			uint16_t &c = count[sd.code];
			if(c == 0){ image[sd.code >> 5] |= 1u << (sd.code & 31); ++distinct; }
			c = (uint16_t)(c + 1 + (inheritors.empty() ? 0 : inheritors[sd.orient].size()));
			if(c > 255){ overflow = true; break; }
			++own[sd.code];
		}
		if(distinct > SEED_MAX_DISTINCT) overflow = true;
		if(!overflow || n_inherited || or_seed.size() < 2) break;
		for(const pcrhost::Seed &sd : seeds){ count[sd.code] = 0; own[sd.code] = 0; }
		std::vector<uint32_t> by_len(or_seed);
		std::stable_sort(by_len.begin(), by_len.end(), [&](uint32_t x, uint32_t y){ return info[x].end - info[x].begin > info[y].end - info[y].begin; });
		const size_t n_drop = (by_len.size() + 3)/4;
		std::vector<uint8_t> drop(n_or, 0);
		for(size_t i = 0;i < n_drop;++i) drop[by_len[i]] = 1;
		std::vector<pcrhost::Seed> kept; kept.reserve(seeds.size());
		for(uint32_t o = 0;o < n_or;++o){
			const uint32_t b = info[o].begin, e = info[o].end;
			info[o].begin = (uint32_t)kept.size();
			if(!drop[o]) kept.insert(kept.end(), seeds.begin() + b, seeds.begin() + e);
			info[o].end = (uint32_t)kept.size();
			if(drop[o]) info[o].seeded = false;
		}
		seeds.swap(kept);
		or_seed.clear(); or_plain.clear();
		for(uint32_t o = 0;o < n_or;++o){ if(info[o].seeded) or_seed.push_back(o); else or_plain.push_back(o); }
	}
	for(const pcrhost::Seed &sd : seeds){
		if(sd.orient & 1u) continue;
		irr_off_mask |= 1u << sd.off;
		if(!inheritors.empty()){ for(const std::pair<uint16_t, int8_t> &in : inheritors[sd.orient]) irr_off_mask |= 1u << (sd.off + in.second); }
	}
	if(overflow){
		or_plain.clear(); or_seed.clear(); image.clear();
		for(uint32_t o = 0;o < n_or;++o) or_plain.push_back(o);
	}
	else{
		uint16_t *rank16 = (uint16_t *)(image.data() + SEED_BITMAP_WORDS);
		uint32_t run = 0;
		for(uint32_t w = 0;w < SEED_BITMAP_WORDS;++w){ rank16[w] = (uint16_t)run; run += (uint32_t)__builtin_popcount(image[w]); }
		heads.assign(distinct, 0u);
		uint32_t n_multi = 0;
		for(const pcrhost::Seed &sd : seeds){
			const uint32_t h = rank16[sd.code >> 5] + (uint32_t)__builtin_popcount(image[sd.code >> 5] & ((1u << (sd.code & 31)) - 1u));
			if(count[sd.code] == 1){ heads[h] = SEED_SINGLE | ((uint32_t)sd.orient << 8) | sd.off; continue; }
			if(heads[h] == 0){ heads[h] = 0x40000000u | n_multi; n_multi += own[sd.code]; }
		}
		std::vector<uint32_t> raw(n_multi, 0u);
		std::vector<uint8_t> &fill = ctx->seed_fill; fill.assign(distinct, 0);
		for(const pcrhost::Seed &sd : seeds){
			if(count[sd.code] == 1) continue;
			const uint32_t h = rank16[sd.code >> 5] + (uint32_t)__builtin_popcount(image[sd.code >> 5] & ((1u << (sd.code & 31)) - 1u));
			const uint32_t start = heads[h] & 0x3FFFFFFFu;
			raw[start + fill[h]++] = (uint32_t)sd.orient | ((uint32_t)sd.off << 24);
		}
		multi.clear(); multi.reserve(n_multi + n_multi/2 + 16);
		for(uint32_t h = 0;h < distinct;++h){
			if(heads[h] & SEED_SINGLE) continue;
			const uint32_t start = heads[h] & 0x3FFFFFFFu, n = fill[h];
			const uint32_t out0 = (uint32_t)multi.size();
			uint32_t header_at = 0, members = 0, cur_base = 0xFFFFFFFFu; int32_t cur_boff = -1;
			for(uint32_t e = 0;e < n;++e){
				const uint32_t sd = raw[start + e], orient = sd & 0xFFFFu, off = sd >> 24;
				const pcrhost::Candidate &c = cand[orient >> 1];
				const int32_t sh = (orient & 1u) ? -c.shift : c.shift;
				int32_t boff = (int32_t)off - sh;
				uint32_t base_orient = 2*c.base + (orient & 1u);
				if(boff < 0 || boff > 24){ boff = (int32_t)off; base_orient = orient; }
				if(members && base_orient == cur_base && boff == cur_boff && members < 256){
					multi.push_back(sd); ++members;
					multi[header_at] = SEED_GROUP | cur_base | ((uint32_t)cur_boff << 16) | ((members - 1) << 21);
				}
				else{
					header_at = (uint32_t)multi.size(); members = 1; cur_base = base_orient; cur_boff = boff;
					multi.push_back(SEED_GROUP | cur_base | ((uint32_t)cur_boff << 16));
					multi.push_back(sd);
				}
				if(!inheritors.empty()){
					for(const std::pair<uint16_t, int8_t> &in : inheritors[orient]){
						if(members == 256){
							header_at = (uint32_t)multi.size(); members = 0;
							multi.push_back(SEED_GROUP | cur_base | ((uint32_t)cur_boff << 16));
						}
						multi.push_back((uint32_t)in.first | ((uint32_t)((int32_t)off + in.second) << 24)); ++members;
						multi[header_at] = SEED_GROUP | cur_base | ((uint32_t)cur_boff << 16) | ((members - 1) << 21);
					}
				}
			}
			heads[h] = (out0 << 9) | ((uint32_t)multi.size() - out0);
		}
		n_multi = (uint32_t)multi.size();
		if(n_multi >= (1u << 22)){ ctx->seed_count.clear(); g_err = "pcr_select_words: seed table too large"; return PCR_ERR_CAPACITY; }
	}
	return PCR_OK;
}


enum class ScanForm { Popcount, BitSliced, Seed1Host, Seed1Dev, Seed2, Seed3 };
inline const char *form_name(ScanForm f)
{
	static const char *const names[] = { "popcount", "bitsliced", "seed1-host", "seed1-dev", "seed2", "seed3" };
	return names[(int)f];
}
inline bool is_seed1(ScanForm f) { return f == ScanForm::Seed1Host || f == ScanForm::Seed1Dev; }
inline bool is_seed2(ScanForm f) { return f == ScanForm::Seed2 || f == ScanForm::Seed3; }

struct ScanPlan {
	ScanForm form = ScanForm::BitSliced;
	std::vector<uint32_t> or_seed, or_plain;
	uint32_t irr_off_mask = 0;
	HostSeedPlan H;
	bool s3_with_irr = false;
	bool need_plain = false, need_seedset = false;
	size_t n_seeds = 0;
	uint32_t n_live = 0, min_len = 0;
	void reset()
	{
		form = ScanForm::BitSliced; or_seed.clear(); or_plain.clear(); irr_off_mask = 0;
		H.seeds.clear(); H.inheritors.clear(); H.n_inherited = 0; H.image.clear(); H.heads.clear(); H.multi.clear();
		s3_with_irr = need_plain = need_seedset = false; n_seeds = 0; n_live = min_len = 0;
	}
};

inline uint32_t live_irregular(const SeqSet &S, uint32_t min_oligo_length)
{
	uint32_t n_live = 0;
	for(uint32_t k = std::min<uint32_t>(min_oligo_length, 256);k < 256;++k) n_live += S.irr_size_count[k];
	return n_live;
}

int irr_index_usable(pcr_ctx *ctx, SeqSet &S, bool &usable)
{
	usable = false;
	if(S.irr_n_multi != 0 || (uint64_t)24*S.n_irr >= (uint64_t(1) << 32)) return PCR_OK;
	const int rc = ensure_irr_index(ctx, S);
	usable = rc == PCR_OK && S.irx_usable;
	return rc;
}

int choose_scan_form(pcr_ctx *ctx, SeqSet &S, const std::vector<pcrhost::Candidate> &cand, int optimize_5, int optimize_3, uint32_t min_oligo_length, ScanPlan &P, PlanLists &L)
{
	const uint32_t n_or = 2*(uint32_t)cand.size();
	std::vector<uint32_t> &or_seed = P.or_seed, &or_plain = P.or_plain;
	P.min_len = min_oligo_length; P.n_live = live_irregular(S, min_oligo_length);
	int rc;
	const bool no_shifts = ctx->scan_version == 3 && !optimize_5 && !optimize_3;
	const bool seed2_ok = no_shifts && !ctx->force_seed1 && n_or <= 65535;
	bool want_seed3 = false;
	if(seed2_ok && !ctx->no_seed3 && !ctx->no_irr_index && ctx->s2_dbg == 0){
		bool worth = true;
		if(!S.pix_valid){
			std::vector<uint32_t> os, op; uint32_t om = 0;
			worth = plan_seed2(ctx, L, cand, os, op, om, nullptr) && op.empty() && !os.empty();
		}
		if(worth){
			if((rc = ensure_pos_index(ctx, S)) != PCR_OK) return rc;
			bool irr_ok = P.n_live == 0;
			if(S.pix_usable && !irr_ok && (rc = irr_index_usable(ctx, S, irr_ok)) != PCR_OK) return rc;
			want_seed3 = S.pix_usable && irr_ok; P.s3_with_irr = P.n_live > 0;
		}
	}
	bool use_seed2 = false;
	if(seed2_ok){
		use_seed2 = plan_seed2(ctx, L, cand, or_seed, or_plain, P.irr_off_mask, want_seed3 ? &S : nullptr);
		if(want_seed3 && !(use_seed2 && or_plain.empty() && !or_seed.empty() && plan_seed3_slices(ctx, L, P.s3_with_irr))){
			or_seed.clear(); or_plain.clear();
			use_seed2 = plan_seed2(ctx, L, cand, or_seed, or_plain, P.irr_off_mask, nullptr);
		}
		if(use_seed2 && !or_plain.empty() && (n_or <= S1_MAX_OR || or_seed.empty())) use_seed2 = false;
		if(!use_seed2){ or_seed.clear(); or_plain.clear(); P.irr_off_mask = 0; }
	}
	const bool use_seed3 = use_seed2 && want_seed3 && or_plain.empty() && !or_seed.empty()
		&& L.s3_prefix.size() == L.s2_seeds.size() + L.s2_group_end.size() && L.s3_spans.size() == L.s2_seeds.size();
	if(use_seed2){ P.form = use_seed3 ? ScanForm::Seed3 : ScanForm::Seed2; P.n_seeds = L.s2_seeds.size(); }
	else if(no_shifts && !ctx->host_seed_tables && n_or <= S1_MAX_OR){
		plan_seed1(ctx, L, cand, or_seed, or_plain, P.irr_off_mask);
		P.form = ScanForm::Seed1Dev; P.n_seeds = L.s1_seeds.size();
	}
	else if(ctx->scan_version == 3 && n_or <= 65535){
		const int prc = plan_seed_host(ctx, cand, P.H, or_seed, or_plain, P.irr_off_mask);
		if(ctx->seed_count.size() == 65536){ for(const pcrhost::Seed &sd : P.H.seeds){ ctx->seed_count[sd.code] = 0; ctx->seed_own[sd.code] = 0; } }
		if(prc != PCR_OK) return prc;
		P.form = ScanForm::Seed1Host; P.n_seeds = P.H.seeds.size() + P.H.n_inherited;
	}
	else{
		for(uint32_t o = 0;o < n_or;++o) or_plain.push_back(o);
		P.form = (ctx->scan_version == 1) ? ScanForm::Popcount : ScanForm::BitSliced;
	}
	if(or_seed.empty() && P.form != ScanForm::Popcount) P.form = ScanForm::BitSliced;
	P.need_plain = (ctx->scan_version != 1) && !or_plain.empty();
	P.need_seedset = !or_seed.empty() && S.n_degen_tiles > 0;
	return PCR_OK;
}

struct PassJob {
	pcr_ctx *ctx = nullptr; int which = 0, opt5 = 0, opt3 = 0; float thr = 0.0f; uint32_t min_len = 0; bool async = false;
	pcr_amplify_args args = {}; FusedAmp fa = {}; bool has_fa = false;
	uint32_t seq = 0;
	bool begun = false, ctrl_was_clean = false;
	std::vector<pcrhost::Candidate> cand; ScanPlan P; PlanLists L;
	std::vector<uint4> hf, hr; std::vector<uint32_t> hfl;
	std::vector<OligoDev> ol;
	bool fuse = false; size_t bits_bytes = 0;
	Seed3HalfSlices pair_W; uint32_t pair_slice_cap = 0;
	void reset()
	{
		seq = 0; begun = ctrl_was_clean = false; has_fa = false; fa = FusedAmp(); async = false;
		cand.clear(); P.reset(); L.clear(); hf.clear(); hr.clear(); hfl.clear(); ol.clear(); fuse = false; bits_bytes = 0;
	}
};

struct Scan2Staged { Scan2Tables T; const uint32_t *d_tab = nullptr, *d_bias = nullptr, *d_map = nullptr; };
struct StagedTables {
	SeedTables ST = {};
	Seed2Tables ST2 = {};
	const uint32_t *d_s3_prefix = nullptr; const uint8_t *d_s3_spans = nullptr;
	Scan2Staged plain, seedset;
	bool lean = false, fuse = false;
	size_t bits_bytes = 0;
};

void stage_scan2(Stager &st, const std::vector<uint32_t> &orients, Scan2Staged &B)
{
	B.d_tab = st.put(B.T.tab.data(), B.T.tab.size());
	B.d_bias = st.put(B.T.bias.data(), B.T.bias.size());
	std::vector<uint32_t> m(orients);
	m.resize((m.size() + 255) & ~size_t(255), 0xFFFFFFFFu);
	B.d_map = st.put(m.data(), m.size());
}

void prepare_tables(const SeqSet &S, PassJob &J, FusedAmp *fa)
{
	const std::vector<pcrhost::Candidate> &cand = J.cand;
	const uint32_t ncand = (uint32_t)cand.size(), n_or = 2*ncand;
	J.hf.resize(ncand); J.hr.resize(ncand); J.hfl.resize(ncand);
	for(uint32_t c = 0;c < ncand;++c){
		J.hf[c] = make_uint4(cand[c].fwd.a, cand[c].fwd.c, cand[c].fwd.g, cand[c].fwd.t);
		J.hr[c] = make_uint4(cand[c].rc.a, cand[c].rc.c, cand[c].rc.g, cand[c].rc.t);
		J.hfl[c] = cand[c].floor_;
	}
	if(is_seed2(J.P.form)){
		std::vector<uint8_t> &floors2 = J.L.s2_floors;
		floors2.assign(((size_t)n_or + 15) & ~size_t(15), 0);
		for(uint32_t o = 0;o < n_or;++o) floors2[o] = (uint8_t)std::min<uint32_t>(cand[o >> 1].floor_, 255u);
	}
	J.fuse = false; J.bits_bytes = 0; J.ol.clear();
	if(fa && fa->n_pairs){
		J.bits_bytes = (size_t)fa->n_pairs*((S.n + 63)/64)*sizeof(uint64_t);
		J.fuse = ((uintptr_t)fa->d_fr % 16 == 0) && ((uintptr_t)fa->d_rf % 16 == 0) && (J.bits_bytes % 16 == 0);
		if(J.fuse) build_oligos(fa->pairs, fa->n_pairs, fa->a, J.ol);
	}
}

int stage_tables(pcr_ctx *ctx, SeqSet &S, const PassJob &J, FusedAmp *fa, bool async, bool ctrl_was_clean, StagedTables &T)
{
	const std::vector<pcrhost::Candidate> &cand = J.cand;
	const ScanPlan &P = J.P; const PlanLists &L = J.L;
	const uint32_t ncand = (uint32_t)cand.size(), n_or = 2*ncand;
	const bool seed2 = is_seed2(P.form), seed3 = P.form == ScanForm::Seed3;
	const bool build_tables = P.form == ScanForm::Seed1Dev;
	const HostSeedPlan &H = P.H;
	int rc;
	if(P.need_plain) build_scan2_tables(cand, P.or_plain, T.plain.T);
	if(P.need_seedset) build_scan2_tables(cand, P.or_seed, T.seedset.T);
	size_t bytes = ncand*(2*sizeof(uint4) + sizeof(uint32_t)) + 1024;
	bytes += (T.plain.T.tab.size() + T.plain.T.bias.size() + P.or_plain.size() + 256)*sizeof(uint32_t);
	bytes += (T.seedset.T.tab.size() + T.seedset.T.bias.size() + P.or_seed.size() + 256)*sizeof(uint32_t);
	bytes += (H.image.size() + H.heads.size() + H.multi.size() + 64)*sizeof(uint32_t);
	if(seed2){
		bytes += L.s2_masks.size()*sizeof(uint4) + L.s2_floors.size() + L.s2_seeds.size()*sizeof(uint32_t) + 512;
		if(seed3) bytes += L.s3_prefix.size()*sizeof(uint32_t) + L.s3_spans.size() + 128;
	}
	if(build_tables) bytes += L.s1_seeds.size()*sizeof(uint32_t) + 256;
	T.bits_bytes = J.bits_bytes; T.fuse = J.fuse;
	if(T.fuse) bytes += J.ol.size()*sizeof(OligoDev) + 64;
	const uint32_t guard_seq = J.seq ? J.seq : ctx->mail_seq + 1;
	const uint64_t gen = S.ctrl.generation;
	if((rc = S.ctrl.ensure(8 + 2*(size_t)S.n + 4)) != PCR_OK) return rc;
	T.lean = ctx->direct_ok && async && T.fuse && seed2 && !P.or_seed.empty() && ctrl_was_clean && gen == S.ctrl.generation
		&& S.bucket_cap == POST_CAP && 2*fa->n_pairs <= 32*POST_MASK_WORDS;
	if(ctx->debug_log) fprintf(stderr, "[pcramp] staging: %s\n", T.lean ? "lean (tables written into device memory, no staging launch)" : "k_stage");
	Stager st(ctx);
	if((rc = T.lean ? st.begin_direct(bytes) : st.begin(bytes)) != PCR_OK) return rc;
	ctx->d_cand_fwd = st.put(J.hf.data(), ncand);
	ctx->d_cand_rc = st.put(J.hr.data(), ncand);
	ctx->d_cand_floor = st.put(J.hfl.data(), ncand);
	if(P.need_plain) stage_scan2(st, P.or_plain, T.plain);
	if(P.need_seedset) stage_scan2(st, P.or_seed, T.seedset);
	if(!H.image.empty()){
		T.ST.image = st.put(H.image.data(), H.image.size());
		T.ST.heads = st.put(H.heads.data(), H.heads.size());
		T.ST.multi = H.multi.empty() ? T.ST.heads : st.put(H.multi.data(), H.multi.size());
	}
	const uint32_t *d_s1_seeds = nullptr;
	if(build_tables){
		d_s1_seeds = st.put(L.s1_seeds.data(), L.s1_seeds.size());
		if((rc = ctx->s1_image.ensure(SEED_IMAGE_WORDS)) != PCR_OK) return rc;
		if((rc = ctx->s1_heads.ensure(2*(size_t)S1_MAX_SEEDS)) != PCR_OK) return rc;
		if((rc = ctx->s1_multi.ensure(S1_MAX_SEEDS)) != PCR_OK) return rc;
		T.ST.image = ctx->s1_image.p; T.ST.heads = ctx->s1_heads.p; T.ST.multi = ctx->s1_multi.p; T.ST.flat = 1;
	}
	if(seed2){
		T.ST2.seeds = st.put(L.s2_seeds.data(), L.s2_seeds.size());
		T.ST2.masks = st.put(reinterpret_cast<const uint4 *>(L.s2_masks.data()), L.s2_masks.size());
		T.ST2.floors = st.put(L.s2_floors.data(), L.s2_floors.size());
		T.ST2.n_seeds = (uint32_t)L.s2_seeds.size(); T.ST2.n_or = n_or;
		if(seed3){ T.d_s3_prefix = st.put(L.s3_prefix.data(), L.s3_prefix.size()); T.d_s3_spans = st.put(L.s3_spans.data(), L.s3_spans.size()); }
	}
	const size_t ctrl_bytes = (8 + 2*(size_t)S.n)*sizeof(uint32_t);
	if(T.fuse){
		fa->d_oligos = st.put(J.ol.data(), J.ol.size());
		fa->staged = true;
		if(T.lean) st.seal(guard_seq);
		else if((rc = st.ship(S.ctrl.p, ctrl_bytes, fa->d_fr, T.bits_bytes, fa->d_rf, T.bits_bytes, guard_seq)) != PCR_OK) return rc;
	}
	else if((rc = st.ship(S.ctrl.p, ctrl_bytes, nullptr, 0, nullptr, 0, guard_seq)) != PCR_OK) return rc;
	if(build_tables){
		if((rc = ctx->s1_part.ensure(2*S1_GROUPS)) != PCR_OK) return rc;
		hipLaunchKernelGGL(k_seed_tables<false>, dim3(S1_GROUPS), dim3(S1_BUILD_THREADS), 0, ctx->stream, d_s1_seeds, (uint32_t)L.s1_seeds.size(),
			ctx->s1_part.p, ctx->s1_image.p, ctx->s1_heads.p, ctx->s1_multi.p);
		hipLaunchKernelGGL(k_seed_tables<true>, dim3(S1_GROUPS), dim3(S1_BUILD_THREADS), 0, ctx->stream, d_s1_seeds, (uint32_t)L.s1_seeds.size(),
			ctx->s1_part.p, ctx->s1_image.p, ctx->s1_heads.p, ctx->s1_multi.p);
		HIP_TRY(hipGetLastError());
	}
	return PCR_OK;
}


int launch_popcount(pcr_ctx *ctx, SeqSet &S, const HitSink &sink)
{
	hipLaunchKernelGGL(k_scan, dim3(S.n_tiles), dim3(SCAN_THREADS), 0, ctx->stream, S.planes.p, S.valid_d(),
		S.d_blk_off.p, S.d_len.p, S.d_active.p, S.tile_seq.p, S.tile_pos0.p, ctx->d_cand_fwd, ctx->d_cand_rc,
		ctx->d_cand_floor, sink.ncand, sink);
	HIP_TRY(hipGetLastError());
	return PCR_OK;
}

int launch_seed1(pcr_ctx *ctx, SeqSet &S, const ScanPlan &P, const StagedTables &T, const HitSink &sink)
{
	const uint32_t ncand = sink.ncand;
	const bool cand_lds = ncand <= SEED_CAND_LDS;
	const auto kernel = cand_lds ? k_seed<true> : k_seed<false>;
	const size_t dyn = cand_lds ? (size_t)ncand*(2*sizeof(uint4) + sizeof(uint32_t)) : 0;
	int per_cu = 0;
	const hipError_t oe = hipOccupancyMaxActiveBlocksPerMultiprocessor(&per_cu, kernel, SEED_THREADS, dyn);
	const size_t lds_wg = ((sizeof(SeedShared) + dyn + 4095)/4096)*4096;
	per_cu = std::max(1, std::min<int>(per_cu, (int)((160*1024)/lds_wg)));
	const uint32_t resident = (oe == hipSuccess) ? (uint32_t)per_cu*ctx->n_cu : SEED_MAX_GRID;
	const uint32_t tiles_per_wg = SEED_WAVES*SEED_TILES_PER_WAVE;
	const dim3 sgrid(std::min<uint32_t>((S.n_tiles + tiles_per_wg - 1)/tiles_per_wg, resident)), sblock(SEED_THREADS);
	IrrArgs IA; IA.irr = S.irr.p; IA.perm = S.irr_perm.p; IA.n_live = P.n_live; IA.off_mask = P.or_plain.empty() ? P.irr_off_mask : 0u;
	const uint32_t irr_wgs = (P.n_live + IRR_THREADS*IRR_PER_LANE - 1)/(IRR_THREADS*IRR_PER_LANE);
	const dim3 fgrid(sgrid.x + irr_wgs);
	if(ctx->debug_log) fprintf(stderr, "[pcramp] k_seed: %d workgroups per CU x %u CUs\n", per_cu, ctx->n_cu);
	hipLaunchKernelGGL(kernel, fgrid, sblock, dyn, ctx->stream, S.tb_d(), S.planes.p, S.valid_d(), S.d_blk_off.p, S.d_nblk_real.p, S.d_len.p, S.d_active.p,
		S.tile_seq.p, S.tile_pos0.p, S.tile_degen.p, S.n_tiles, T.ST, ctx->d_cand_fwd, ctx->d_cand_rc, ctx->d_cand_floor, ncand, IA, sgrid.x, sink);
	HIP_TRY(hipGetLastError());
	return PCR_OK;
}

void seed3_args(SeqSet &S, const Seed2Tables &Tg, const uint32_t *d_chunk_prefix, const uint8_t *d_spans, const pcr_ctx::S3Launch &L3, const IrrArgs2 &IA, Seed3Tables &T3, Seed3Set &Q3)
{
	T3.seeds = Tg.seeds; T3.spans = d_spans; T3.chunk_prefix = d_chunk_prefix; T3.masks = Tg.masks; T3.floors = Tg.floors;
	T3.n_seeds = Tg.n_seeds; T3.n_or = Tg.n_or; T3.or_base = Tg.or_base;
	T3.pix_first = S.pix_first.p; T3.pix_last = S.pix_last.p; T3.pix_ent = S.pix_ent.p;
	Q3 = Seed3Set{ S.valid_d(), S.blk_info.p, S.blk_local.p, S.d_active.p };
	T3.n_chunks = L3.n_chunks; T3.per_wg = L3.per_wg; T3.slice_cap = L3.slice_cap;
	T3.n_irr_wg = IA.ix_first ? L3.n_irr_wg : 0u;
}
inline size_t seed3_lds(const Seed3Tables &T3)
{
	return (size_t)T3.n_or*sizeof(uint4) + 2*(size_t)T3.slice_cap*sizeof(uint32_t) + (((size_t)T3.n_or + 15) & ~size_t(15)) + (((size_t)T3.slice_cap + 15) & ~size_t(15)) + 16;
}

int launch_seed3_group(pcr_ctx *ctx, SeqSet &S, const Seed2Tables &Tg, const uint32_t *d_chunk_prefix, const uint8_t *d_spans, const pcr_ctx::S3Launch &L3, const IrrArgs2 &IA,
	const HitSink &sink, const S2Clear &Z)
{
	Seed3Tables T3; Seed3Set Q3;
	seed3_args(S, Tg, d_chunk_prefix, d_spans, L3, IA, T3, Q3);
	const size_t dyn3 = seed3_lds(T3);
	if(!ctx->s3_attr_set){
		HIP_TRY(hipFuncSetAttribute((const void *)k_seed3<S3_WG_THREADS>, hipFuncAttributeMaxDynamicSharedMemorySize, 128*1024));
		ctx->s3_attr_set = true;
	}
	hipLaunchKernelGGL(k_seed3<S3_WG_THREADS>, dim3(seed3_grid(ctx)), dim3(S3_WG_THREADS), dyn3, ctx->stream, T3, Q3, IA, ctx->d_cand_fwd, ctx->d_cand_floor, sink, Z, L3.W);
	return PCR_OK;
}

IrrArgs2 group_irr_args(SeqSet &S, const ScanPlan &P, uint32_t group_offmask, bool first_launch, bool irr_by_index)
{
	IrrArgs2 IA; IA.scan = S.irr_scan.p; IA.irr = S.irr.p; IA.n_live = P.n_live;
	IA.off_mask = group_offmask;
	IA.exhaustive = first_launch ? 1u : 0u;
	IA.ix_first = IA.ix_last = IA.ix_words = nullptr; IA.min_cws = std::min<uint32_t>(P.min_len, 255u);
	if(!P.or_plain.empty()){
		IA.off_mask = 0;
		if(!first_launch) IA.n_live = 0;
	}
	else if(irr_by_index){
		IA.ix_first = S.irx_first.p; IA.ix_last = S.irx_last.p; IA.ix_words = S.irx_words.p; IA.n_live = 0;
	}
	return IA;
}
S2Clear group_clear(const StagedTables &T, const FusedAmp *fa, const HitSink &sink, bool first_launch)
{
	S2Clear Z = { nullptr, 0u, nullptr, 0u, nullptr };
	if(T.lean && first_launch){
		Z.z0 = (uint4 *)fa->d_fr; Z.z1 = (uint4 *)fa->d_rf; Z.n0 = Z.n1 = (uint32_t)(T.bits_bytes/16); Z.ctrl = sink.counters;
	}
	return Z;
}

int launch_seed_groups(pcr_ctx *ctx, SeqSet &S, const ScanPlan &P, const PlanLists &L, const StagedTables &T, const FusedAmp *fa, const HitSink &sink)
{
	const bool seed3 = P.form == ScanForm::Seed3;
	const uint32_t tiles_per_wg = S2_WAVES*2;
	const dim3 sgrid(std::max<uint32_t>(1u, std::min<uint32_t>((S.n_tiles + tiles_per_wg - 1)/tiles_per_wg, ctx->n_cu))), sblock(S2_THREADS);
	int rc;
	if(!ctx->s2_attr_set){
		HIP_TRY(hipFuncSetAttribute((const void *)k_seed2<false>, hipFuncAttributeMaxDynamicSharedMemorySize, (int)(160*1024 - sizeof(S2Shared))));
		HIP_TRY(hipFuncSetAttribute((const void *)k_seed2<true>, hipFuncAttributeMaxDynamicSharedMemorySize, (int)(160*1024 - sizeof(S2Shared))));
		ctx->s2_attr_set = true;
	}
	const auto k_seed2_of_ctx = ctx->s2_dbg ? k_seed2<true> : k_seed2<false>;
	bool irr_by_index = P.s3_with_irr;
	if(!seed3){
		irr_by_index = P.or_plain.empty() && P.n_live > 0 && !ctx->no_irr_index;
		for(size_t g = 0, b = 0;g < L.s2_group_end.size();++g){ if((size_t)L.s2_group_end[g] - b > (size_t)sgrid.x*S2_THREADS) irr_by_index = false; b = L.s2_group_end[g]; }
		if(irr_by_index && (rc = irr_index_usable(ctx, S, irr_by_index)) != PCR_OK) return rc;
	}
	uint32_t g_begin = 0, g_prefix = 0;
	bool first_launch = true;
	for(size_t g = 0;g < L.s2_group_end.size();++g){
		Seed2Tables Tg = T.ST2;
		const uint32_t or0 = L.s2_group_or[g], g_or = L.s2_group_nor[g];
		const uint8_t *const d_spans = seed3 ? T.d_s3_spans + g_begin : nullptr;
		Tg.seeds = T.ST2.seeds + g_begin; Tg.n_seeds = L.s2_group_end[g] - g_begin;
		Tg.masks = T.ST2.masks + (size_t)or0; Tg.floors = T.ST2.floors + or0; Tg.n_or = g_or; Tg.or_base = or0;
		g_begin = L.s2_group_end[g];
		if(Tg.n_seeds == 0){ g_prefix += 1u; continue; }
		const size_t dyn = (size_t)g_or*sizeof(uint4) + (((size_t)g_or + 15) & ~size_t(15)) + 8*((size_t)Tg.n_seeds + 64) + 16;
		const IrrArgs2 IA = group_irr_args(S, P, L.s2_group_offmask[g], first_launch, irr_by_index);
		if(ctx->debug_log) fprintf(stderr, "[pcramp] k_seed2: %u workgroups, %u seeds of orientations %u..%u (group %zu of %zu), %zu + %zu B of LDS\n", sgrid.x, Tg.n_seeds,
			or0, or0 + g_or - 1, g + 1, L.s2_group_end.size(), sizeof(S2Shared), dyn);
		const S2Clear Z = group_clear(T, fa, sink, first_launch);
		if(seed3){
			if((rc = launch_seed3_group(ctx, S, Tg, T.d_s3_prefix + g_prefix, d_spans, L.s3_launch[g], IA, sink, Z)) != PCR_OK) return rc;
			g_prefix += Tg.n_seeds + 1u;
		}
		else hipLaunchKernelGGL(k_seed2_of_ctx, sgrid, sblock, dyn, ctx->stream, S.tb_d(), S.valid_d(), S.tile_desc.p, S.n_tiles, Tg, S.d_active.p, ctx->d_cand_fwd, ctx->d_cand_floor,
			sink.ncand, IA, sink, ctx->s2_dbg, Z);
		HIP_TRY(hipGetLastError());
		first_launch = false;
	}
	return PCR_OK;
}

int launch_irregular(pcr_ctx *ctx, SeqSet &S, const ScanPlan &P, const HitSink &sink)
{
	const unsigned irr_grid = (P.n_live + IRR_THREADS*IRR_PER_LANE - 1)/(IRR_THREADS*IRR_PER_LANE);
	hipLaunchKernelGGL(k_scan_irr, dim3(irr_grid), dim3(IRR_THREADS), 0, ctx->stream, S.irr.p, S.irr_perm.p, P.n_live,
		S.d_active.p, ctx->d_cand_fwd, ctx->d_cand_floor, sink.ncand, sink);
	HIP_TRY(hipGetLastError());
	return PCR_OK;
}

int launch_scans(pcr_ctx *ctx, SeqSet &S, const ScanPlan &P, const PlanLists &L, const StagedTables &T, const FusedAmp *fa, const HitSink &sink)
{
	int rc = PCR_OK;
	const uint32_t ncand = sink.ncand;
	if(S.n_tiles){
		ProfScope scan_prof(ctx, PCR_PROF_SCAN, ctx->prof && (ctx->prof_pass++ % ctx->prof_stride) == 0);
		if(P.need_plain && (rc = launch_scan2(ctx, S, T.plain.T, ncand, sink, T.plain.d_tab, T.plain.d_bias, nullptr, S.n_tiles, T.plain.d_map)) != PCR_OK) return rc;
		if(P.form == ScanForm::Popcount) rc = launch_popcount(ctx, S, sink);
		else if(is_seed1(P.form)) rc = launch_seed1(ctx, S, P, T, sink);
		else if(is_seed2(P.form)) rc = launch_seed_groups(ctx, S, P, L, T, fa, sink);
		if(rc != PCR_OK) return rc;
		if(P.need_seedset && (rc = launch_scan2(ctx, S, T.seedset.T, ncand, sink, T.seedset.d_tab, T.seedset.d_bias, S.degen_tiles.p, S.n_degen_tiles,
			T.seedset.d_map)) != PCR_OK) return rc;
		scan_prof.finish();
	}
	const bool irr_taken = S.n_tiles && (is_seed1(P.form) || is_seed2(P.form));
	if(P.n_live && !irr_taken) rc = launch_irregular(ctx, S, P, sink);
	return rc;
}


PostRow post_row_args(pcr_ctx *ctx, SeqSet &S, const HitSink &sink, const FusedAmp *fa, uint32_t seq)
{
	PostRow R;
	R.hits = sink.hits; R.seq_count = sink.seq_count; R.best = sink.best; R.ncand = sink.ncand; R.planes = S.planes.p; R.blk_off = S.d_blk_off.p;
	R.irr = S.irr.p; R.irr_off = S.irr_off.p; R.db = S.db.p; R.seg_hi = S.d_seg_hi; R.counters = sink.counters; R.epoch = sink.epoch; R.n_seq = S.n;
	R.oligos = fa->d_oligos; R.n_pairs = fa->n_pairs; R.mask_words = (2*fa->n_pairs + 31)/32; R.len = S.d_len.p; R.active = S.d_active.p;
	R.amp_min = fa->a->amp_min; R.amp_max = fa->a->amp_max; R.ident_thr = fa->a->ident_threshold; R.use_taq = fa->a->use_taq_mama;
	R.bits_fr = fa->d_fr; R.bits_rf = fa->d_rf; R.bit_words = (uint64_t)((S.n + 63)/64); R.pub_mail = ctx->mail.dev + (seq % pcr_ctx::MAIL_RING); R.pub_seq = seq;
	return R;
}
template<class K>
void launch_post(K kernel, uint32_t waves, pcr_ctx *ctx, SeqSet &S, const HitSink &sink, const FusedAmp *fa, uint32_t seq)
{
	const PostRow R = post_row_args(ctx, S, sink, fa, seq);
	hipLaunchKernelGGL(kernel, dim3((S.n + waves - 1)/waves), dim3(64*waves), 0, ctx->stream, R.hits, R.seq_count, R.best, R.ncand, R.planes,
		R.blk_off, R.irr, R.irr_off, R.db, R.seg_hi, R.counters, R.epoch, R.n_seq,
		R.oligos, R.n_pairs, R.mask_words, R.len, R.active, R.amp_min, R.amp_max,
		R.ident_thr, R.use_taq, R.bits_fr, R.bits_rf, R.bit_words, R.pub_mail, R.pub_seq);
}
int fused_tail(pcr_ctx *ctx, SeqSet &S, const HitSink &sink, FusedAmp *fa, uint32_t reserved_seq)
{
	const uint32_t seq = reserved_seq ? reserved_seq : ++ctx->mail_seq;
	if(sink.cap == POST_CAP){
		launch_post(k_post<8>, 8, ctx, S, sink, fa, seq);
		S.ctrl_clean = true; S.touched_from_seg = true;
	}
	else if(sink.cap == 128) launch_post(k_post_big<128, 4>, 4, ctx, S, sink, fa, seq);
	else launch_post(k_post_big<256, 4>, 4, ctx, S, sink, fa, seq);
	HIP_TRY(hipGetLastError());
	fa->posted = true;
	S.touched_built = false;
	return PCR_OK;
}

template<class K, class... Extra>
void launch_finalize(K kernel, dim3 grid, dim3 block, size_t lds, pcr_ctx *ctx, SeqSet &S, const HitSink &sink, Extra... extra)
{
	hipLaunchKernelGGL(kernel, grid, block, lds, ctx->stream, sink.hits, sink.seq_count, sink.cap, sink.best, sink.ncand, S.planes.p, S.d_blk_off.p, S.irr.p,
		S.irr_off.p, S.db.p, S.d_seg_hi, sink.counters, sink.epoch, S.touched.p, extra...);
}
template<bool ALL = false>
int plain_tail(pcr_ctx *ctx, SeqSet &S, const HitSink &sink, bool async, FusedAmp *fa)
{
	int rc;
	hipLaunchKernelGGL(k_touched, dim3((S.n + 255)/256), dim3(256), 0, ctx->stream, sink.seq_count, S.n, sink.counters, S.touched.p);
	HIP_TRY(hipGetLastError());
	S.touched_built = true;
	uint32_t np2 = 1; while(np2 < sink.cap) np2 <<= 1;
	if(np2 <= 1024) launch_finalize(k_finalize<FIN_WAVES, ALL>, dim3((S.n + FIN_WAVES - 1)/FIN_WAVES), dim3(64*FIN_WAVES), (size_t)FIN_WAVES*np2*sizeof(uint64_t), ctx, S, sink);
	else if(np2 <= MAX_BUCKET_CAP) launch_finalize(k_finalize<1, ALL>, dim3(S.n), dim3(64), (size_t)np2*sizeof(uint64_t), ctx, S, sink);
	else{
		if((rc = ctx->fin_scratch.ensure((size_t)S.n*np2)) != PCR_OK) return rc;
		launch_finalize(k_finalize_big<ALL>, dim3(S.n), dim3(FINBIG_THREADS), 0, ctx, S, sink, ctx->fin_scratch.p);
	}
	HIP_TRY(hipGetLastError());
	++ctx->mail_seq;
	if(async && fa && fa->staged){ fa->pub_seq = ctx->mail_seq; fa->pub_counters = sink.counters; }
	else{
		hipLaunchKernelGGL(k_publish, dim3(1), dim3(64), 0, ctx->stream, sink.counters, ctx->mail.dev + (ctx->mail_seq % pcr_ctx::MAIL_RING), ctx->mail_seq);
		HIP_TRY(hipGetLastError());
	}
	return PCR_OK;
}

uint32_t resized_buckets(bool overflowed, uint32_t cap, uint32_t largest_fill, int attempt)
{
	if(overflowed){
		uint32_t want = cap*2;
		while(want < largest_fill && want < MAX_BUCKET_CAP_GLOBAL) want *= 2;
		return want;
	}
	if(cap <= 64 || attempt >= 12) return 0;
	uint32_t want = 64;
	while(want < largest_fill + largest_fill/16) want *= 2;
	return (want*4 <= cap) ? want : 0;
}

inline bool fused_tail_fits(uint32_t cap, uint32_t n_pairs) { return (cap == POST_CAP || cap == 128 || cap == 256) && 2*n_pairs <= 32*POST_MASK_WORDS; }
inline bool buckets_fit(uint64_t n_slots) { return n_slots < (uint64_t(1) << 32) && n_slots*(sizeof(Hit) + sizeof(DevEntry)) <= (uint64_t(96) << 30); }

inline bool begin_pass(SeqSet &S)
{
	S.have_db = false; S.n_entries = 0;
	const bool ctrl_was_clean = S.ctrl_clean;
	S.ctrl_clean = false; S.touched_from_seg = false;
	return ctrl_was_clean;
}

int plan_pass(pcr_ctx *ctx, PassJob &J, const pcr_pair *pairs, uint32_t n_pairs)
{
	SeqSet &S = ctx->sets[J.which];
	HostTimer timer(ctx, 0);
	if(ctx->timing) ++ctx->n_timed;
	pcrhost::build_candidates((const uint64_t *)pairs, n_pairs, J.opt5 != 0, J.opt3 != 0, J.thr, J.cand);
	const uint32_t ncand = (uint32_t)J.cand.size();
	if(S.n == 0 || ncand == 0) return PCR_OK;
	int rc;
	if((rc = choose_scan_form(ctx, S, J.cand, J.opt5, J.opt3, J.min_len, J.P, J.L)) != PCR_OK) return rc;
	if(ctx->debug_log) fprintf(stderr, "[pcramp] scan plan: form=%s, %u candidates, %zu seeded orientations (%zu seeds), %zu plain, %u/%u IUPAC tiles, %u-slot buckets\n",
		form_name(J.P.form), ncand, J.P.or_seed.size(), J.P.n_seeds, J.P.or_plain.size(), S.n_degen_tiles, S.n_tiles, S.bucket_cap);
	prepare_tables(S, J, J.has_fa ? &J.fa : nullptr);
	return PCR_OK;
}

bool plans_without_device_work(const pcr_ctx *ctx, const SeqSet &S, int opt5, int opt3, uint32_t min_len)
{
	if(ctx->scan_version != 3 || opt5 || opt3 || ctx->force_seed1) return false;
	const bool may_want_seed3 = !ctx->no_seed3 && !ctx->no_irr_index && ctx->s2_dbg == 0;
	if(may_want_seed3 && !S.pix_valid) return false;
	if(live_irregular(S, min_len) == 0 || ctx->no_irr_index) return true;
	return S.irr_n_multi != 0 || (uint64_t)24*S.n_irr >= (uint64_t(1) << 32) || S.irx_valid;
}

bool pass_is_pipelinable(const pcr_ctx *ctx, const PassJob &J)
{
	const SeqSet &S = ctx->sets[J.which];
	return J.async && J.has_fa && J.fuse && S.n != 0 && !J.cand.empty() && is_seed2(J.P.form)
		&& fused_tail_fits(S.bucket_cap, J.fa.n_pairs) && buckets_fit((uint64_t)S.n*S.bucket_cap);
}


int stage_pass(pcr_ctx *ctx, PassJob &J, bool ctrl_was_clean, StagedTables &T)
{
	SeqSet &S = ctx->sets[J.which];
	int rc;
	if((rc = ctx->best.ensure((size_t)S.n*J.cand.size())) != PCR_OK) return rc;
	if(ctx->best.generation != ctx->best_seen){
		HIP_TRY(hipMemsetAsync(ctx->best.p, 0, ctx->best.cap*sizeof(uint32_t), ctx->stream));
		ctx->best_seen = ctx->best.generation; ctx->epoch = std::min(ctx->debug_epoch, EPOCH_LIMIT);
	}
	if((rc = stage_tables(ctx, S, J, J.has_fa ? &J.fa : nullptr, J.async, ctrl_was_clean, T)) != PCR_OK) return rc;
	if((rc = S.touched.ensure(S.n)) != PCR_OK) return rc;
	S.d_seg_hi = S.ctrl.p + 8 + S.n;
	return PCR_OK;
}

int size_attempt(pcr_ctx *ctx, SeqSet &S, const PassJob &J, int attempt, HitSink &sink)
{
	int rc;
	const uint32_t cap = S.bucket_cap;
	const uint64_t n_slots = (uint64_t)S.n*cap;
	if(!buckets_fit(n_slots)){
		assert(J.seq == 0);
		S.bucket_cap = 64;
		g_err = "pcr_select_words: the per-sequence hit buckets would not fit (too many tied sites per sequence)"; return PCR_ERR_CAPACITY;
	}
	if((rc = ctx->hits.ensure(n_slots)) != PCR_OK) return rc;
	if((rc = S.db.ensure(n_slots)) != PCR_OK) return rc;
	if(attempt > 0) HIP_TRY(hipMemsetAsync(S.ctrl.p, 0, (8 + 2*(size_t)S.n)*sizeof(uint32_t), ctx->stream));
	if(ctx->epoch >= EPOCH_LIMIT){
		HIP_TRY(hipMemsetAsync(ctx->best.p, 0, ctx->best.cap*sizeof(uint32_t), ctx->stream));
		ctx->epoch = 0;
	}
	++ctx->epoch;
	sink.best = ctx->best.p; sink.hits = ctx->hits.p; sink.seq_count = S.ctrl.p + 8;
	sink.counters = S.ctrl.p; sink.cap = cap; sink.ncand = (uint32_t)J.cand.size(); sink.epoch = ctx->epoch;
	return PCR_OK;
}

inline void pass_enqueued(SeqSet &S, uint32_t cap)
{
	S.db_cap = cap; S.n_slots = (uint64_t)S.n*cap;
	S.n_touched = N_TOUCHED_UNKNOWN; S.n_entries = 1; S.have_db = true;
}

int run_pass(pcr_ctx *ctx, PassJob &J, uint64_t *n_entries_out)
{
	SeqSet &S = ctx->sets[J.which];
	FusedAmp *const fa = J.has_fa ? &J.fa : nullptr;
	const bool async = J.async;
	const bool ctrl_was_clean = J.begun ? J.ctrl_was_clean : begin_pass(S);
	const ScanPlan &P = J.P;
	const uint32_t ncand = (uint32_t)J.cand.size();
	if(S.n == 0 || ncand == 0){ S.have_db = true; S.n_touched = 0; return PCR_OK; }
	HostTimer timer(ctx, 1);
	int rc;
	StagedTables T;
	if((rc = stage_pass(ctx, J, ctrl_was_clean, T)) != PCR_OK) return rc;

	timer.next(2);
	uint32_t h_counters[4];
	for(int attempt = 0;;++attempt){
		const uint32_t cap = S.bucket_cap;
		const uint64_t n_slots = (uint64_t)S.n*cap;
		HitSink sink;
		if((rc = size_attempt(ctx, S, J, attempt, sink)) != PCR_OK) return rc;
		const bool fused = async && fa && fa->staged && fused_tail_fits(cap, fa->n_pairs);
		if(J.seq && !fused){ g_err = "pcr_screen_device: a pipelined pass lost its fused tail"; return PCR_ERR_STATE; }
		if((rc = launch_scans(ctx, S, P, J.L, T, fa, sink)) != PCR_OK) return rc;
		if((rc = fused ? fused_tail(ctx, S, sink, fa, J.seq) : plain_tail(ctx, S, sink, async, fa)) != PCR_OK) return rc;
		if(async){ pass_enqueued(S, cap); return PCR_OK; }
		timer.next(3);
		if((rc = mail_wait(ctx, ctx->mail_seq, h_counters)) != PCR_OK) return rc;
		timer.next(2);
		S.db_cap = cap; S.n_slots = n_slots;
		const bool overflowed = (h_counters[0] & 1u) != 0;
		if(overflowed && (attempt >= 12 || cap >= MAX_BUCKET_CAP_GLOBAL)){ g_err = "pcr_select_words: more than 65536 candidate sites in one sequence (per-sequence bucket limit)"; return PCR_ERR_CAPACITY; }
		const uint32_t want = resized_buckets(overflowed, cap, h_counters[2], attempt);
		if(!want) break;
		S.bucket_cap = want;
	}
	if(ctx->debug_log) fprintf(stderr, "[pcramp] pass done: %u-slot buckets, largest fill %u, %u sequences with entries\n", S.db_cap, h_counters[2], h_counters[3]);
	S.n_touched = h_counters[3];
	S.n_entries = S.n_touched ? 1 : 0;
	S.have_db = true;
	if(n_entries_out){
		if((rc = count_entries(ctx, S)) != PCR_OK) return rc;
		*n_entries_out = S.n_entries;
	}
	return PCR_OK;
}


bool pass_is_pairable(const pcr_ctx *ctx, const PassJob &J)
{
	const SeqSet &S = ctx->sets[J.which];
	return ctx->pair_mode != 0 && pass_is_pipelinable(ctx, J) && J.P.form == ScanForm::Seed3 && J.L.s2_group_end.size() == 1 && J.L.s2_group_end[0] != 0
		&& !J.P.need_plain && !J.P.need_seedset && S.n_tiles != 0 && S.bucket_cap == POST_CAP
		&& !(ctx->prof && ctx->prof_pass % ctx->prof_stride == 0);
}

bool pair_slices(const pcr_ctx *ctx, PassJob &J)
{
	const pcr_ctx::S3Launch &L3 = J.L.s3_launch[0];
	const uint32_t ns = J.L.s2_group_end[0], G = (seed3_grid(ctx) - L3.n_irr_wg) & ~1u, Gh = G/2;
	uint32_t *const st = J.pair_W.start;
	for(uint32_t w = 0;w <= Gh;++w) st[w] = L3.W.start[2*w];
	for(uint32_t w = Gh + 1;w <= S3_MAX_WG/2;++w) st[w] = st[Gh];
	uint32_t cap = 2;
	for(uint32_t w = 0;w < Gh;++w) cap = std::max(cap, std::min(st[w + 1] + 2u, ns + 1u) - st[w]);
	J.pair_slice_cap = cap;
	return 17*(size_t)J.L.s2_group_nor[0] + 9*(size_t)cap + 64 <= S3_LDS_BUDGET;
}

bool passes_can_pair(PassJob &A, PassJob &B)
{
	if(A.ctx == B.ctx || !pass_is_pairable(A.ctx, A) || !pass_is_pairable(B.ctx, B)) return false;
	const uintptr_t a[2] = { (uintptr_t)A.fa.d_fr, (uintptr_t)A.fa.d_rf }, b[2] = { (uintptr_t)B.fa.d_fr, (uintptr_t)B.fa.d_rf };
	for(int i = 0;i < 2;++i) for(int j = 0;j < 2;++j){ if(a[i] < b[j] + B.bits_bytes && b[j] < a[i] + A.bits_bytes) return false; }
	return pair_slices(A.ctx, A) && pair_slices(B.ctx, B);
}

struct PairHalf { pcr_ctx *ctx; PassJob *J; SeqSet *S; StagedTables T; HitSink sink; Seed3Row scan; PostRow post; };
int prepare_half(PairHalf &H)
{
	pcr_ctx *const ctx = H.ctx; PassJob &J = *H.J; SeqSet &S = *H.S;
	const bool ctrl_was_clean = begin_pass(S);
	int rc;
	HostTimer timer(ctx, 1);
	if((rc = stage_pass(ctx, J, ctrl_was_clean, H.T)) != PCR_OK) return rc;
	timer.next(2);
	if((rc = size_attempt(ctx, S, J, 0, H.sink)) != PCR_OK) return rc;
	if(!J.fa.staged || H.sink.cap != POST_CAP){ g_err = "pcr_screen_device: a paired pass lost its fused tail"; return PCR_ERR_STATE; }
	if(ctx->prof) ++ctx->prof_pass;
	const PlanLists &L = J.L;
	Seed2Tables Tg = H.T.ST2;
	Tg.n_seeds = L.s2_group_end[0]; Tg.masks = H.T.ST2.masks + (size_t)L.s2_group_or[0]; Tg.floors = H.T.ST2.floors + L.s2_group_or[0];
	Tg.n_or = L.s2_group_nor[0]; Tg.or_base = L.s2_group_or[0];
	H.scan.IA = group_irr_args(S, J.P, L.s2_group_offmask[0], true, J.P.s3_with_irr);
	seed3_args(S, Tg, H.T.d_s3_prefix, H.T.d_s3_spans, L.s3_launch[0], H.scan.IA, H.scan.T3, H.scan.Q);
	H.scan.T3.per_wg *= 2u; H.scan.T3.slice_cap = J.pair_slice_cap; H.scan.T3.n_irr_wg = (H.scan.T3.n_irr_wg + 1u)/2u;
	H.scan.cand_fwd = ctx->d_cand_fwd; H.scan.cand_floor = ctx->d_cand_floor; H.scan.sink = H.sink;
	H.scan.Z = group_clear(H.T, &J.fa, H.sink, true);
	H.post = post_row_args(ctx, S, H.sink, &J.fa, J.seq);
	return PCR_OK;
}

int run_pass_pair(PassJob &JA, PassJob &JB)
{
	PairHalf H[2];
	H[0].ctx = JA.ctx; H[0].J = &JA; H[1].ctx = JB.ctx; H[1].J = &JB;
	int rc;
	for(PairHalf &h : H){
		h.S = &h.ctx->sets[h.J->which];
		if((rc = prepare_half(h)) != PCR_OK) return rc;
	}
	pcr_ctx *const ctx = JA.ctx;
	HostTimer timer(ctx, 2);
	const uint32_t Gx = seed3_grid(ctx)/2;
	const size_t dyn3 = std::max(seed3_lds(H[0].scan.T3), seed3_lds(H[1].scan.T3));
	if(!ctx->s3_pair_attr_set){
		HIP_TRY(hipFuncSetAttribute((const void *)k_seed3_pair<S3_WG_THREADS>, hipFuncAttributeMaxDynamicSharedMemorySize, 128*1024));
		ctx->s3_pair_attr_set = true;
	}
	const uint32_t Px = (std::max(H[0].S->n, H[1].S->n) + 7u)/8u;
	if(ctx->debug_log) fprintf(stderr, "[pcramp] paired launch: passes %u + %u, scan grid %u x 2 (irregular workgroups %u + %u, slice_cap' %u + %u, %zu B of LDS), tail grid %u x 2\n",
		JA.seq, JB.seq, Gx, H[0].scan.T3.n_irr_wg, H[1].scan.T3.n_irr_wg, H[0].scan.T3.slice_cap, H[1].scan.T3.slice_cap, dyn3, Px);
	hipLaunchKernelGGL(k_seed3_pair<S3_WG_THREADS>, dim3(Gx, 2), dim3(S3_WG_THREADS), dyn3, ctx->stream, H[0].scan, JA.pair_W, H[1].scan, JB.pair_W);
	HIP_TRY(hipGetLastError());
	hipLaunchKernelGGL(k_post_pair<8>, dim3(Px, 2), dim3(64*8), 0, ctx->stream, H[0].post, H[1].post);
	HIP_TRY(hipGetLastError());
	for(PairHalf &h : H){
		h.S->ctrl_clean = true; h.S->touched_from_seg = true;
		h.J->fa.posted = true; h.S->touched_built = false;
		pass_enqueued(*h.S, POST_CAP);
	}
	return PCR_OK;
}

void fill_job(pcr_ctx *ctx, PassJob &J, pcr_set which, int optimize_5, int optimize_3, float threshold, uint32_t min_oligo_length, bool async, const FusedAmp *fa)
{
	J.ctx = ctx; J.which = (int)which; J.opt5 = optimize_5; J.opt3 = optimize_3; J.thr = threshold; J.min_len = min_oligo_length; J.async = async;
	J.has_fa = fa != nullptr;
	if(fa){ J.fa = *fa; J.args = *fa->a; J.fa.a = &J.args; }
}

void quiesce_stream(pcr_ctx *ctx);

int select_impl(pcr_ctx *ctx, pcr_set which, const pcr_pair *pairs, uint32_t n_pairs, int optimize_5, int optimize_3,
	float threshold, uint32_t min_oligo_length, uint64_t *n_entries_out, bool async, FusedAmp *fa = nullptr)
{
	if(!ctx || (n_pairs && !pairs)){ g_err = "pcr_select_words: bad argument"; return PCR_ERR_ARG; }
	if(min_oligo_length < 1 || min_oligo_length > 32){ g_err = "pcr_select_words: min_oligo_length must be in [1,32]"; return PCR_ERR_ARG; }
	HIP_TRY(hipSetDevice(ctx->device));
	if(n_entries_out) *n_entries_out = 0;
	assert(ctx->lq_client.queued.load() == 0);
	quiesce_stream(ctx);
	PassJob J;
	fill_job(ctx, J, which, optimize_5, optimize_3, threshold, min_oligo_length, async, fa);
	J.ctrl_was_clean = begin_pass(ctx->sets[which]); J.begun = true;
	int rc = plan_pass(ctx, J, pairs, n_pairs);
	if(rc == PCR_OK) rc = run_pass(ctx, J, n_entries_out);
	if(fa){ const pcr_amplify_args *a = fa->a; *fa = J.fa; fa->a = a; }
	return rc;
}


struct Launcher {
	int device; hipStream_t stream; unsigned refs = 0;
	cpu_set_t near; bool have_near = false;
	struct InFlight { const pcr_ctx *ctx; const PassMail *slot; uint32_t seq; };
	std::mutex inflight_m; std::vector<InFlight> inflight;
	pcrq::LaunchQueue q;
	Launcher(int dev, hipStream_t st, unsigned spin_us);
	void forget_published()
	{
		inflight.erase(std::remove_if(inflight.begin(), inflight.end(), [](const InFlight &f){
			const uint32_t v = __atomic_load_n((const uint32_t *)&f.slot->seq, __ATOMIC_ACQUIRE);
			return v >= f.seq && (v - f.seq) % pcr_ctx::MAIL_RING == 0; }), inflight.end());
	}
	void launched(const PassJob &J)
	{
		std::lock_guard<std::mutex> lk(inflight_m);
		if(inflight.size() >= 4*pcr_ctx::MAIL_RING){ forget_published(); if(inflight.size() >= 4*pcr_ctx::MAIL_RING) inflight.erase(inflight.begin()); }
		inflight.push_back(InFlight{ J.ctx, J.ctx->mail.host + (J.seq % pcr_ctx::MAIL_RING), J.seq });
	}
	size_t backlog()
	{
		std::lock_guard<std::mutex> lk(inflight_m);
		forget_published();
		return inflight.size();
	}
	void forget_handle(const pcr_ctx *ctx)
	{
		std::lock_guard<std::mutex> lk(inflight_m);
		inflight.erase(std::remove_if(inflight.begin(), inflight.end(), [&](const InFlight &f){ return f.ctx == ctx; }), inflight.end());
	}
};
constexpr unsigned PAIR_HOLD_CAP_US = 20000;
std::mutex g_launchers_m;
std::vector<Launcher *> g_launchers;

PassJob *acquire_job(pcr_ctx *ctx)
{
	PassJob *J = nullptr;
	{
		std::lock_guard<std::mutex> lk(ctx->job_m);
		if(!ctx->job_free.empty()){ J = ctx->job_free.back(); ctx->job_free.pop_back(); }
	}
	if(!J){ J = new PassJob(); ctx->job_all.push_back(J); }
	return J;
}
void release_job(pcr_ctx *ctx, PassJob *J)
{
	J->reset();
	std::lock_guard<std::mutex> lk(ctx->job_m);
	ctx->job_free.push_back(J);
}
void free_jobs(pcr_ctx *ctx)
{
	for(PassJob *J : ctx->job_all) delete J;
	ctx->job_all.clear(); ctx->job_free.clear();
}

constexpr unsigned LAUNCH_SPIN_US = 200;

bool read_cpu_list(const std::string &path, cpu_set_t &set)
{
	CPU_ZERO(&set);
	FILE *f = fopen(path.c_str(), "r");
	if(!f) return false;
	char buf[4096]; const bool got = fgets(buf, sizeof(buf), f) != nullptr;
	fclose(f);
	if(!got) return false;
	for(const char *p = buf;*p && *p != '\n';){
		char *e; const long a = strtol(p, &e, 10);
		if(e == p) return false;
		long b = a;
		if(*e == '-'){ p = e + 1; b = strtol(p, &e, 10); if(e == p) return false; }
		for(long c = a;c <= b && c < CPU_SETSIZE;++c) CPU_SET((int)c, &set);
		p = (*e == ',') ? e + 1 : e;
	}
	return true;
}
bool near_cpus(cpu_set_t &out)
{
	const int cpu = sched_getcpu();
	if(cpu < 0) return false;
	const std::string base = "/sys/devices/system/cpu/cpu" + std::to_string(cpu);
	cpu_set_t llc, core, allowed;
	if(!read_cpu_list(base + "/cache/index3/shared_cpu_list", llc)) return false;
	if(!read_cpu_list(base + "/topology/thread_siblings_list", core)) CPU_ZERO(&core);
	CPU_SET(cpu, &core);
// ... 187 lines not shown
```

Before: 26.47 billion.

## Keep seed lists resident on device and stage slices from compact records

```diff
diff --git a/pcramp_amd/csrc/pcr_device.hip b/pcramp_amd/csrc/pcr_device.hip
--- a/pcramp_amd/csrc/pcr_device.hip
+++ b/pcramp_amd/csrc/pcr_device.hip
@@ -640,7 +640,7 @@
 	struct S2KeyHash { size_t operator()(const S2Key &k) const { uint64_t h = 0x9E3779B97F4A7C15ull; for(uint32_t v : {k.a, k.c, k.g, k.t, k.floor_}){ h ^= v; h *= 0x100000001B3ull; h ^= h >> 29; } return (size_t)h; } };
 	struct S2Entry { std::vector<uint32_t> seeds;  uint32_t off_mask; bool seedable; };
 	std::vector<pcrhost::Seed> s2_tmp;
-	struct S3Launch { Seed3Slices W; uint32_t n_chunks, per_wg, slice_cap, n_irr_wg; };
+	struct S3Launch { Seed3Slices W; uint32_t n_chunks, per_wg, slice_cap, n_irr_wg, rec_cap; };
 	int pair_mode = 1; bool s3_pair_attr_set = false;
 	bool no_seed3 = false, s3_attr_set = false;
 	bool s3_next = true;
@@ -736,6 +736,9 @@
 	DevBuf<pcr_pool_dimer_end3> pde3_rec, pde3_out; DevBuf<pcr_dimer_placement> pde3_place;
 	bool pde3_attr_set = false;
 	DevBuf<pcr_pool_dimer_end3> pcx_dense; DevBuf<pcr_pool_conflict_ext> pcx_rec, pcx_out;
+	bool s3_resident = true;
+	size_t seed_store_bytes = size_t(32) << 20;
+	DevBuf<uint32_t> seed_store_buf{true}; pcrseed::Store seed_store; bool seed_store_failed = false; uint64_t seed_store_resets = 0;
 };
 
 namespace {
@@ -1339,6 +1342,8 @@
 	if(const char *v = getenv("PCRAMP_IRR_INDEX")) ctx->no_irr_index = v[0] == '0';
 	if(const char *v = getenv("PCRAMP_SEED3")) ctx->no_seed3 = v[0] == '0';
 	if(const char *v = getenv("PCRAMP_S3_NEXT")) ctx->s3_next = v[0] != '0';
+	if(const char *v = getenv("PCRAMP_S3_RESIDENT")) ctx->s3_resident = v[0] != '0';
+	if(const char *v = getenv("PCRAMP_DEBUG_SEED_STORE")) ctx->seed_store_bytes = std::max<size_t>(4096, (size_t)strtoull(v, nullptr, 0));
 	if(const char *v = getenv("PCRAMP_SEED_MEMO")) ctx->seed_lists.use_memo = v[0] != '0';
 	if(const char *v = getenv("PCRAMP_LAUNCH_THREAD")) ctx->launch_thread = v[0] != '0';
 	if(const char *v = getenv("PCRAMP_PAIR")) ctx->pair_mode = (v[0] == '0') ? 0 : (strcmp(v, "force") == 0) ? 2 : 1;
diff --git a/pcramp_amd/csrc/pcr_scan_seed3.inc b/pcramp_amd/csrc/pcr_scan_seed3.inc
--- a/pcramp_amd/csrc/pcr_scan_seed3.inc
+++ b/pcramp_amd/csrc/pcr_scan_seed3.inc
@@ -32,11 +32,14 @@
 }
 
 struct Seed3Tables {
-	const uint32_t *seeds;
-	const uint32_t *chunk_prefix;
+	union { const uint32_t *seeds;
+	        const uint32_t *store; };
+	union { const uint32_t *chunk_prefix;
+	        const uint4 *records; };
 	const uint8_t *spans;
 	const uint4 *masks; const uint8_t *floors;
-	uint32_t n_seeds, n_or, or_base;
+	union { uint32_t n_seeds; uint32_t n_rec; }; uint32_t n_or, or_base;
+	uint32_t rec_cap;
 	const uint32_t *pix_first, *pix_last; const uint4 *pix_ent;
 	uint32_t n_chunks, per_wg, slice_cap;
 	uint32_t n_irr_wg;
@@ -102,6 +105,41 @@
 	}
 }
 
+__device__ __forceinline__ void s3_irregular_rec(const Seed3Tables &T3, const Seed3Set &Q, const IrrArgs2 &IA, const uint4 *__restrict__ cand_fwd,
+	const uint32_t *__restrict__ cand_floor, HitSink sink, uint32_t gw, uint32_t n_gw, uint32_t lane)
+{
+	for(uint32_t r = gw;r < T3.n_rec;r += n_gw){
+		const uint4 rec = T3.records[r];
+		const uint32_t n = rec.z & 0xFFFFu, orient = T3.or_base + (rec.z >> 16), c = orient >> 1;
+		if(orient & 1u) continue;
+		const uint32_t floor_c = cand_floor[c]; const uint4 fwd_c = cand_fwd[c];
+		for(uint32_t k0 = 0;k0 < n;k0 += 64u){
+			const uint32_t k = k0 + lane;
+			uint32_t first = 0, cnt = 0;
+			if(k < n){
+				const uint32_t sdv = T3.store[rec.x + k];
+				const uint32_t key = (((sdv >> 9) & 31u) << 18) | (sdv >> 14);
+				first = IA.ix_first[key]; cnt = IA.ix_last[key] - first;
+			}
+			const uint32_t incl = s2_scan(cnt);
+			const uint32_t total = s2_rl(incl, 63);
+			for(uint32_t t0 = 0;t0 < total;t0 += 64u){
+				const uint32_t t = t0 + lane;
+				uint32_t lo = 0;
+#pragma unroll
+				for(uint32_t stp = 32u;stp;stp >>= 1){ if((uint32_t)__shfl((int)incl, (int)(lo + stp - 1u)) <= t) lo += stp; }
+				const int sl = (int)min(lo, 63u);
+				const uint32_t s_incl = (uint32_t)__shfl((int)incl, sl), s_cnt = (uint32_t)__shfl((int)cnt, sl), s_first = (uint32_t)__shfl((int)first, sl);
+				if(t >= total) continue;
+				const IrrDev e = IA.irr[IA.ix_words[s_first + (t - (s_incl - s_cnt))]];
+				if(((e.meta >> 8) & 0xFFu) < IA.min_cws || !Q.active[e.seq]) continue;
+				const uint32_t nm = match_count(e.w.a, e.w.c, e.w.g, e.w.t, fwd_c);
+				if(nm >= floor_c) record_hit(sink, e.seq, c, make_key(e.seq, e.loc, e.meta & 0xFF, 1, (e.meta >> 16) & 0xFF), nm);
+			}
+		}
+	}
+}
+
 template<uint32_t S3_THREADS>
 __global__ __launch_bounds__(S3_THREADS) __attribute__((amdgpu_waves_per_eu(8, 8))) void k_seed3(Seed3Tables T3, Seed3Set Q, IrrArgs2 IA, const uint4 *__restrict__ cand_fwd, const uint32_t *__restrict__ cand_floor,
 	HitSink sink, S2Clear Z, Seed3Slices W)
diff --git a/pcramp_amd/csrc/pcr_scan_seed3_pass.inc b/pcramp_amd/csrc/pcr_scan_seed3_pass.inc
--- a/pcramp_amd/csrc/pcr_scan_seed3_pass.inc
+++ b/pcramp_amd/csrc/pcr_scan_seed3_pass.inc
@@ -1,9 +1,11 @@
 	extern __shared__ uint4 s3_dyn[];
+	const bool resident = T3.rec_cap != 0u;
 	uint4 *const masks = s3_dyn;
 	uint32_t *const prefix = (uint32_t *)(masks + T3.n_or);
 	uint32_t *const seeds = prefix + T3.slice_cap;
 	uint8_t *const floors = (uint8_t *)(seeds + T3.slice_cap);
 	uint8_t *const spans = floors + ((T3.n_or + 15u) & ~15u);
+	uint2 *const bounds = (uint2 *)spans;
 	const uint32_t wave = (uint32_t)__builtin_amdgcn_readfirstlane((int)(threadIdx.x >> 6)), lane = threadIdx.x & 63u;
 	for(uint32_t i = blockIdx.x*S3_THREADS + threadIdx.x;i < Z.n0;i += gridDim.x*S3_THREADS) Z.z0[i] = make_uint4(0, 0, 0, 0);
 	for(uint32_t i = blockIdx.x*S3_THREADS + threadIdx.x;i < Z.n1;i += gridDim.x*S3_THREADS) Z.z1[i] = make_uint4(0, 0, 0, 0);
@@ -11,13 +13,38 @@
 	for(uint32_t i = threadIdx.x;i < T3.n_or;i += S3_THREADS){ masks[i] = T3.masks[i]; floors[i] = T3.floors[i]; }
 	constexpr uint32_t S3_WAVES = S3_THREADS/64;
 	if(blockIdx.x < T3.n_irr_wg){
-		if(IA.ix_first) s3_irregular(T3, Q, IA, cand_fwd, cand_floor, sink, blockIdx.x*S3_WAVES + wave, T3.n_irr_wg*S3_WAVES, lane);
+		if(IA.ix_first){
+			if(resident) s3_irregular_rec(T3, Q, IA, cand_fwd, cand_floor, sink, blockIdx.x*S3_WAVES + wave, T3.n_irr_wg*S3_WAVES, lane);
+			else s3_irregular(T3, Q, IA, cand_fwd, cand_floor, sink, blockIdx.x*S3_WAVES + wave, T3.n_irr_wg*S3_WAVES, lane);
+		}
 		return;
 	}
 	const uint32_t wg = blockIdx.x - T3.n_irr_wg, n_wg = gridDim.x - T3.n_irr_wg;
 	const uint32_t s_lo = W.start[wg];
-	const uint32_t n_slice = min(min(W.start[wg + 1] + 2u, T3.n_seeds + 1u) - s_lo, T3.slice_cap);
-	for(uint32_t i = threadIdx.x;i < n_slice;i += S3_THREADS){ prefix[i] = T3.chunk_prefix[s_lo + i]; const bool in = s_lo + i < T3.n_seeds; seeds[i] = in ? T3.seeds[s_lo + i] : 0u; spans[i] = in ? T3.spans[s_lo + i] : (uint8_t)0; }
+	uint32_t n_slice;
+	if(resident){
+		uint4 *const recs = (uint4 *)(bounds + ((T3.slice_cap + 1u) & ~1u));
+		const uint32_t n_r = min(min(W.start[wg + 1], T3.n_rec - 1u) - s_lo + 2u, T3.rec_cap);
+		for(uint32_t i = threadIdx.x;i < n_r;i += S3_THREADS) recs[i] = T3.records[s_lo + i];
+		__syncthreads();
+		uint32_t n_stage = 0;
+		for(uint32_t j = 0;j + 1u < n_r;++j) n_stage += recs[j].z & 0xFFFFu;
+		n_stage = min(n_stage, T3.slice_cap - 1u);
+		for(uint32_t t = threadIdx.x;t < n_stage;t += S3_THREADS){
+			uint32_t j = 0, k = t;
+			while(k >= (recs[j].z & 0xFFFFu)){ k -= recs[j].z & 0xFFFFu; ++j; }
+			const uint4 r = recs[j];
+			const uint32_t n = r.z & 0xFFFFu;
+			const uint32_t *__restrict__ const sl = T3.store + r.y;
+			prefix[t] = r.w + sl[k]; seeds[t] = T3.store[r.x + k] | (r.z >> 16); bounds[t] = make_uint2(sl[n + k], sl[2u*n + k]);
+		}
+		if(threadIdx.x == 0){ prefix[n_stage] = recs[n_r - 1u].w; seeds[n_stage] = 0u; bounds[n_stage] = make_uint2(0u, 0u); }
+		n_slice = n_stage + 1u;
+	}
+	else{
+		n_slice = min(min(W.start[wg + 1] + 2u, T3.n_seeds + 1u) - s_lo, T3.slice_cap);
+		for(uint32_t i = threadIdx.x;i < n_slice;i += S3_THREADS){ prefix[i] = T3.chunk_prefix[s_lo + i]; const bool in = s_lo + i < T3.n_seeds; seeds[i] = in ? T3.seeds[s_lo + i] : 0u; spans[i] = in ? T3.spans[s_lo + i] : (uint8_t)0; }
+	}
 	__syncthreads();
 	const uint32_t gw = wg*S3_WAVES + wave, n_gw = n_wg*S3_WAVES;
 	const uint32_t q_lo = wg*T3.per_wg, q_hi = min(q_lo + T3.per_wg, T3.n_chunks);
@@ -29,9 +56,13 @@
 				uint32_t lo = 0, hi = n_slice - 1u;
 				while(hi - lo > 1u){ const uint32_t mid = (lo + hi) >> 1; if(prefix[mid] <= q) lo = mid; else hi = mid; }
 				c_sd = seeds[lo];
-				const uint32_t key = (c_sd >> 14) << 2, sp = spans[lo];
-				const uint32_t f = T3.pix_first[key + (sp & 3u)], e = T3.pix_last[key + (sp >> 2)], j0 = (q - prefix[lo])*64u;
-				c_first = f + j0; c_cnt = (e - f) - j0;
+				const uint32_t j0 = (q - prefix[lo])*64u;
+				if(resident){ const uint2 fl = bounds[lo]; c_first = fl.x + j0; c_cnt = fl.y - j0; }
+				else{
+					const uint32_t key = (c_sd >> 14) << 2, sp = spans[lo];
+					const uint32_t f = T3.pix_first[key + (sp & 3u)], e = T3.pix_last[key + (sp >> 2)];
+					c_first = f + j0; c_cnt = (e - f) - j0;
+				}
 			}
 		}
 		uint4 en[S3_BATCH];
@@ -76,4 +107,7 @@
 			else record_hit(sink, seq, c, make_key(seq, (int32_t)p_local, 1, 0, 0), cnt_b[b]);
 		}
 	}
-	if(IA.ix_first && T3.n_irr_wg == 0) s3_irregular(T3, Q, IA, cand_fwd, cand_floor, sink, gw, n_gw, lane);
+	if(IA.ix_first && T3.n_irr_wg == 0){
+		if(resident) s3_irregular_rec(T3, Q, IA, cand_fwd, cand_floor, sink, gw, n_gw, lane);
+		else s3_irregular(T3, Q, IA, cand_fwd, cand_floor, sink, gw, n_gw, lane);
+	}
diff --git a/pcramp_amd/csrc/pcr_seed_lists.hpp b/pcramp_amd/csrc/pcr_seed_lists.hpp
--- a/pcramp_amd/csrc/pcr_seed_lists.hpp
+++ b/pcramp_amd/csrc/pcr_seed_lists.hpp
@@ -59,6 +59,8 @@
 	Mask16 mask = {0, 0, 0, 0}; uint32_t off_mask = 0, n = 0; bool seedable = false;
 	uint32_t next_slot = 0, total[CHUNK_SETS] = {0, 0, 0, 0}; uint64_t gen[CHUNK_SETS] = {0, 0, 0, 0};
 	uint32_t *block = nullptr;
+	uint32_t dev_seeds = 0, dev_seeds_epoch = 0, dev_slot[CHUNK_SETS] = {0, 0, 0, 0}, dev_slot_epoch[CHUNK_SETS] = {0, 0, 0, 0};
+	uint64_t dev_slot_gen[CHUNK_SETS] = {0, 0, 0, 0};
 };
 struct Entry : EntryHead {
 	Entry() {}
@@ -88,6 +90,19 @@
 
 struct Limits { uint32_t max_or, max_seeds; size_t lds_fixed, lds_budget; uint32_t max_groups; };
 
+struct Store {
+	uint32_t *base = nullptr; size_t cap_words = 0, used = 0; uint32_t epoch = 1; bool wrote = false;
+	bool alloc(size_t words, uint32_t &off)
+	{
+		words = (words + 3) & ~size_t(3);
+		if(!base || used + words > cap_words) return false;
+		off = (uint32_t)used; used += words; return true;
+	}
+	void reset() { used = 0; ++epoch; if(epoch == 0) epoch = 1; }
+};
+
+struct Rec16 { uint32_t seeds_off, slot_off, n_tag, pf_base; };
+
 struct Lister {
 	Cache second, third;
 	size_t clear_above = 16384;
@@ -102,6 +117,7 @@
 	std::vector<uint32_t> s2_group_end, s2_group_offmask, s2_group_or, s2_group_nor;
 	RawBuf<uint32_t> s3_prefix;
 	RawBuf<uint8_t> s3_spans;
+	RawBuf<Rec16> s3_records; std::vector<uint32_t> s3_rec_end; bool s3_resident = false;
 };
 
 inline Entry *derive(Lister &Z, Cache &C, const Key &key, const Planes &m, bool third, bool fold)
@@ -241,6 +257,132 @@
 	return true;
 }
 
+
+inline bool upload_seeds(Entry &e, Store &D)
+{
+	if(e.dev_seeds_epoch == D.epoch) return true;
+	uint32_t off;
+	if(!D.alloc(e.n, off)) return false;
+	uint32_t *__restrict out = D.base + off; const uint32_t *__restrict sd = e.seeds();
+	for(uint32_t k = 0;k < e.n;++k) out[k] = sd[k];
+	e.dev_seeds = off; e.dev_seeds_epoch = D.epoch; D.wrote = true;
+	return true;
+}
+inline bool upload_slot(Entry &e, int s, const SetIndex &S, Store &D)
+{
+	if(e.dev_slot_epoch[s] == D.epoch && e.dev_slot_gen[s] == S.generation) return true;
+	uint32_t off;
+	if(!D.alloc(3*(size_t)e.n, off)) return false;
+	const uint32_t n = e.n;
+	uint32_t *__restrict o_run = D.base + off, *__restrict o_first = o_run + n, *__restrict o_len = o_first + n;
+	const uint32_t *__restrict sd = e.seeds(), *__restrict run = e.run(s); const uint8_t *__restrict sp = e.spans();
+	for(uint32_t k = 0;k < n;++k){
+		const uint32_t key4 = (sd[k] >> 14) << 2, span = sp[k], f = S.start[key4 + (span & 3u)];
+		o_run[k] = run[k]; o_first[k] = f; o_len[k] = S.start[key4 + (span >> 2) + 1u] - f;
+	}
+	e.dev_slot[s] = off; e.dev_slot_epoch[s] = D.epoch; e.dev_slot_gen[s] = S.generation; D.wrote = true;
+	return true;
+}
+
+enum class Listed { Ok, NoFit, StoreFull };
+
+inline Listed list_records(Lister &Z, Store &D, const Limits &lim, const pcrhost::Candidate *cand, size_t n_cand, const SetIndex &S3, bool fold,
+	SeedLists &L, std::vector<uint32_t> &or_seed, std::vector<uint32_t> &or_plain, uint32_t &irr_off_mask)
+{
+	const uint32_t n_or = 2*(uint32_t)n_cand;
+	L.s2_seeds.clear(); L.s3_prefix.clear(); L.s3_spans.clear(); L.s3_records.clear(); L.s3_rec_end.clear(); L.s3_resident = false;
+	L.s2_group_end.clear(); L.s2_group_offmask.clear(); L.s2_group_or.clear(); L.s2_group_nor.clear();
+	irr_off_mask = 0;
+	if(Z.second.map.size() > Z.clear_above) Z.second.clear();
+	if(Z.third.map.size() > Z.clear_above){
+		if(D.used) return Listed::StoreFull;
+		Z.third.clear();
+	}
+	L.s2_masks.resize(n_or);
+	Cache &C = Z.third;
+	if(Z.use_memo && C.memo.size() < n_or) C.memo.resize(n_or, Cache::Slot{Key{0, 0, 0, 0, 0}, nullptr});
+	auto fits = [&lim](size_t n, uint32_t g_or){ return g_or <= lim.max_or && n <= lim.max_seeds && lim.lds_fixed + 17*(size_t)g_or + 8*n <= lim.lds_budget; };
+	auto push = [&L](const Rec16 &r){ const size_t i = L.s3_records.size(); L.s3_records.resize(i + 1); L.s3_records[i] = r; };
+	size_t n_out = 0, group_begin = 0; uint32_t group_mask = 0, group_or0 = 0, group_last = 0, pf_run = 0;
+	Mask16 *const masks = L.s2_masks.data();
+	for(uint32_t o = 0;o < n_or;++o){
+		const pcrhost::Candidate &c = cand[o >> 1];
+		const Planes &m = (o & 1u) ? c.rc : c.fwd;
+		const Key key = {m.a, m.c, m.g, m.t, c.floor_};
+		Entry *e;
+		Cache::Slot *const memo = Z.use_memo ? &C.memo[o] : nullptr;
+		if(memo && memo->e && memo->key == key) e = memo->e;
+		else{
+			auto it = C.map.find(key);
+			e = it != C.map.end() ? &it->second : derive(Z, C, key, m, true, fold);
+			if(memo){ memo->key = key; memo->e = e; }
+		}
+		masks[o] = e->mask;
+		if(!e->seedable){ or_plain.push_back(o); continue; }
+		or_seed.push_back(o);
+		if(!fits(n_out - group_begin + e->n, o - group_or0 + 1)){
+			if(!fits(e->n, 1) || L.s2_group_end.size() + 1 >= lim.max_groups) return Listed::NoFit;
+			L.s2_group_end.push_back((uint32_t)n_out); L.s2_group_offmask.push_back(group_mask); L.s2_group_or.push_back(group_or0); L.s2_group_nor.push_back(group_last - group_or0 + 1);
+			push(Rec16{0, 0, 0, pf_run}); L.s3_rec_end.push_back((uint32_t)L.s3_records.size());
+			group_begin = n_out; group_mask = 0; group_or0 = o; pf_run = 0;
+		}
+		group_last = o;
+		const int s = chunk_slot(*e, S3);
+		if(!upload_seeds(*e, D) || !upload_slot(*e, s, S3, D)) return Listed::StoreFull;
+		push(Rec16{e->dev_seeds, e->dev_slot[s], e->n | ((o - group_or0) << 16), pf_run});
+		pf_run += e->total[s];
+		n_out += e->n;
+		if(!(o & 1u)){ irr_off_mask |= e->off_mask; group_mask |= e->off_mask; }
+	}
+	L.s2_group_end.push_back((uint32_t)n_out); L.s2_group_offmask.push_back(group_mask); L.s2_group_or.push_back(group_or0);
+	L.s2_group_nor.push_back(or_seed.empty() ? 0u : group_last - group_or0 + 1);
+	push(Rec16{0, 0, 0, pf_run}); L.s3_rec_end.push_back((uint32_t)L.s3_records.size());
+	L.s3_resident = true;
+	return Listed::Ok;
+}
+
+inline void record_slice_caps(const Rec16 *R, uint32_t nr, const uint32_t *start, uint32_t G, uint32_t &slice_cap, uint32_t &rec_cap)
+{
+	slice_cap = 2; rec_cap = 2;
+	for(uint32_t w = 0;w < G;++w){
+		const uint32_t lo = start[w], hi = std::min(start[w + 1], nr - 1u);
+		uint32_t n = 0;
+		for(uint32_t r = lo;r <= hi;++r) n += R[r].n_tag & 0xFFFFu;
+		slice_cap = std::max(slice_cap, n + 1u); rec_cap = std::max(rec_cap, hi - lo + 2u);
+	}
+	slice_cap = (slice_cap + 1u) & ~1u;
+}
+inline size_t record_lds(uint32_t g_or, uint32_t slice_cap, uint32_t rec_cap) { return 17*(size_t)g_or + 16*(size_t)slice_cap + 16*(size_t)rec_cap + 64; }
+
+template<class Launch>
+inline bool plan_record_slices(const SeedLists &PL, std::vector<Launch> &launch, uint32_t G_all, uint32_t seeds_per_turn, uint32_t max_wg, size_t lds_budget, bool with_irr)
+{
+	launch.resize(PL.s2_group_end.size());
+	size_t g_begin = 0, r0 = 0;
+	for(size_t g = 0;g < PL.s2_group_end.size();++g){
+		const uint32_t ns = PL.s2_group_end[g] - (uint32_t)g_begin;
+		g_begin = PL.s2_group_end[g];
+		const Rec16 *R = PL.s3_records.data() + r0;
+		const uint32_t nr = PL.s3_rec_end[g] - (uint32_t)r0 - 1u;
+		r0 = PL.s3_rec_end[g];
+		Launch &L = launch[g];
+		L.n_irr_wg = with_irr ? std::min<uint32_t>((ns + seeds_per_turn - 1u)/seeds_per_turn, G_all/4u) : 0u;
+		const uint32_t G = (G_all - L.n_irr_wg) & ~1u;
+		L.n_chunks = R[nr].pf_base; L.per_wg = std::max<uint32_t>(1u, (L.n_chunks + G - 1u)/G); L.slice_cap = 2; L.rec_cap = 2;
+		if(ns == 0) continue;
+		uint32_t at = 0;
+		for(uint32_t w = 0;w <= G;++w){
+			const uint64_t target = (uint64_t)w*L.per_wg;
+			while(at + 1u < nr && R[at + 1u].pf_base <= target) ++at;
+			L.W.start[w] = at;
+		}
+		for(uint32_t w = G + 1;w <= max_wg;++w) L.W.start[w] = at;
+		record_slice_caps(R, nr, L.W.start, G, L.slice_cap, L.rec_cap);
+		if(record_lds(PL.s2_group_nor[g], L.slice_cap, L.rec_cap) > lds_budget) return false;
+	}
+	return true;
+}
+
 }
 
 #endif
diff --git a/pcramp_amd/csrc/pcr_select.inc b/pcramp_amd/csrc/pcr_select.inc
--- a/pcramp_amd/csrc/pcr_select.inc
+++ b/pcramp_amd/csrc/pcr_select.inc
@@ -8,6 +8,7 @@
 	{
 		s2_seeds.clear(); s2_masks.clear(); s2_floors.clear(); s2_group_end.clear(); s2_group_offmask.clear(); s2_group_or.clear(); s2_group_nor.clear();
 		s3_launch.clear(); s3_prefix.clear(); s3_spans.clear(); s1_seeds.clear();
+		s3_records.clear(); s3_rec_end.clear(); s3_resident = false;
 	}
 };
 
@@ -33,7 +34,49 @@
 {
 	return pcrseed::plan_slices(PL, PL.s3_launch, seed3_grid(ctx), 16u*(S3_WG_THREADS/64), S3_MAX_WG, S3_LDS_BUDGET, with_irr);
 }
-
+bool plan_seed3_record_slices(pcr_ctx *ctx, PlanLists &PL, bool with_irr)
+{
+	return pcrseed::plan_record_slices(PL, PL.s3_launch, seed3_grid(ctx), 16u*(S3_WG_THREADS/64), S3_MAX_WG, S3_LDS_BUDGET, with_irr);
+}
+
+
+bool seed_store_ready(pcr_ctx *ctx)
+{
+	if(!ctx->s3_resident || !ctx->direct_ok || ctx->seed_store_failed) return false;
+	if(ctx->seed_store.base) return true;
+	const std::string err_before = g_err;
+	const size_t words = std::min<size_t>(ctx->seed_store_bytes/sizeof(uint32_t), 0xFFFFFFF0u);
+	if(ctx->seed_store_buf.ensure(words) != PCR_OK){ (void)hipGetLastError(); g_err = err_before; ctx->seed_store_failed = true; return false; }
+	ctx->seed_store.base = ctx->seed_store_buf.p; ctx->seed_store.cap_words = words;
+	return true;
+}
+int reset_seed_store(pcr_ctx *ctx)
+{
+	int rc;
+	if((rc = flush_launcher(ctx)) != PCR_OK) return rc;
+	if((rc = wait_published(ctx, ctx->mail_seq)) != PCR_OK) return rc;
+	if(ctx->debug_log) fprintf(stderr, "[pcramp] seed store reset: %zu of %zu words used under epoch %u\n", ctx->seed_store.used, ctx->seed_store.cap_words, ctx->seed_store.epoch);
+	ctx->seed_store.reset(); ++ctx->seed_store_resets;
+	return PCR_OK;
+}
+int plan_seed3_resident(pcr_ctx *ctx, PlanLists &L, const std::vector<pcrhost::Candidate> &cand, std::vector<uint32_t> &or_seed, std::vector<uint32_t> &or_plain,
+	uint32_t &irr_off_mask, const SeqSet &S, bool &listed)
+{
+	listed = false;
+	const pcrseed::Limits lim = { S3_MAX_OR, 65535u, 0, ~size_t(0), S2_MAX_GROUPS };
+	const pcrseed::SetIndex ix = { S.pix_start_h.data(), S.pix_generation };
+	for(int attempt = 0;attempt < 2;++attempt){
+		or_seed.clear(); or_plain.clear();
+		const pcrseed::Listed r = pcrseed::list_records(ctx->seed_lists, ctx->seed_store, lim, cand.data(), cand.size(), ix, ctx->s3_next, L, or_seed, or_plain, irr_off_mask);
+		if(ctx->seed_store.wrote){ __builtin_ia32_sfence(); ctx->seed_store.wrote = false; }
+		if(r == pcrseed::Listed::Ok){ listed = true; return PCR_OK; }
+		if(r == pcrseed::Listed::NoFit) return PCR_OK;
+		if(attempt == 1){ ctx->seed_store_failed = true; return PCR_OK; }
+		const int rc = reset_seed_store(ctx);
+		if(rc != PCR_OK) return rc;
+	}
+	return PCR_OK;
+}
 void plan_seed1(pcr_ctx *ctx, PlanLists &L, const std::vector<pcrhost::Candidate> &cand, std::vector<uint32_t> &or_seed, std::vector<uint32_t> &or_plain, uint32_t &irr_off_mask)
 {
 	const uint32_t n_or = 2*(uint32_t)cand.size();
@@ -285,7 +328,14 @@
 		}
 	}
 	bool use_seed2 = false;
-	if(seed2_ok){
+	bool resident = false;
+	if(seed2_ok && want_seed3 && seed_store_ready(ctx)){
+		if((rc = plan_seed3_resident(ctx, L, cand, or_seed, or_plain, P.irr_off_mask, S, resident)) != PCR_OK) return rc;
+		if(resident && !(or_plain.empty() && !or_seed.empty() && plan_seed3_record_slices(ctx, L, P.s3_with_irr))) resident = false;
+		if(!resident){ or_seed.clear(); or_plain.clear(); L.s3_records.clear(); L.s3_rec_end.clear(); L.s3_resident = false; }
+	}
+	if(resident) use_seed2 = true;
+	else if(seed2_ok){
 		use_seed2 = plan_seed2(ctx, L, cand, or_seed, or_plain, P.irr_off_mask, want_seed3 ? &S : nullptr);
 		if(want_seed3 && !(use_seed2 && or_plain.empty() && !or_seed.empty() && plan_seed3_slices(ctx, L, P.s3_with_irr))){
 			or_seed.clear(); or_plain.clear();
@@ -295,8 +345,11 @@
 		if(!use_seed2){ or_seed.clear(); or_plain.clear(); P.irr_off_mask = 0; }
 	}
 	const bool use_seed3 = use_seed2 && want_seed3 && or_plain.empty() && !or_seed.empty()
-		&& L.s3_prefix.size() == L.s2_seeds.size() + L.s2_group_end.size() && L.s3_spans.size() == L.s2_seeds.size();
-	if(use_seed2){ P.form = use_seed3 ? ScanForm::Seed3 : ScanForm::Seed2; P.n_seeds = L.s2_seeds.size(); }
+		&& (L.s3_resident ? L.s3_rec_end.size() == L.s2_group_end.size()
+		                  : L.s3_prefix.size() == L.s2_seeds.size() + L.s2_group_end.size() && L.s3_spans.size() == L.s2_seeds.size());
+	if(use_seed3 && L.s3_resident && ctx->debug_log) fprintf(stderr, "[pcramp] resident plan: %zu records in %zu groups, seed store %zu of %zu words under epoch %u\n",
+		L.s3_records.size() - L.s3_rec_end.size(), L.s3_rec_end.size(), ctx->seed_store.used, ctx->seed_store.cap_words, ctx->seed_store.epoch);
+	if(use_seed2){ P.form = use_seed3 ? ScanForm::Seed3 : ScanForm::Seed2; P.n_seeds = L.s3_resident ? (size_t)L.s2_group_end.back() : L.s2_seeds.size(); }
 	else if(no_shifts && !ctx->host_seed_tables && n_or <= S1_MAX_OR){
 		plan_seed1(ctx, L, cand, or_seed, or_plain, P.irr_off_mask);
 		P.form = ScanForm::Seed1Dev; P.n_seeds = L.s1_seeds.size();
@@ -326,7 +379,7 @@
 	std::vector<uint4> hf, hr; std::vector<uint32_t> hfl;
 	std::vector<OligoDev> ol;
 	bool fuse = false; size_t bits_bytes = 0;
-	Seed3HalfSlices pair_W; uint32_t pair_slice_cap = 0;
+	Seed3HalfSlices pair_W; uint32_t pair_slice_cap = 0, pair_rec_cap = 0;
 	void reset()
 	{
 		seq = 0; begun = ctrl_was_clean = false; has_fa = false; fa = FusedAmp(); async = false;
@@ -339,6 +392,7 @@
 	SeedTables ST = {};
 	Seed2Tables ST2 = {};
 	const uint32_t *d_s3_prefix = nullptr; const uint8_t *d_s3_spans = nullptr;
+	const uint4 *d_s3_records = nullptr; const uint32_t *d_s3_store = nullptr;
 	Scan2Staged plain, seedset;
 	bool lean = false, fuse = false;
 	size_t bits_bytes = 0;
@@ -393,7 +447,7 @@
 	bytes += (H.image.size() + H.heads.size() + H.multi.size() + 64)*sizeof(uint32_t);
 	if(seed2){
 		bytes += L.s2_masks.size()*sizeof(uint4) + L.s2_floors.size() + L.s2_seeds.size()*sizeof(uint32_t) + 512;
-		if(seed3) bytes += L.s3_prefix.size()*sizeof(uint32_t) + L.s3_spans.size() + 128;
+		if(seed3) bytes += L.s3_prefix.size()*sizeof(uint32_t) + L.s3_spans.size() + L.s3_records.size()*sizeof(uint4) + 128;
 	}
 	if(build_tables) bytes += L.s1_seeds.size()*sizeof(uint32_t) + 256;
 	T.bits_bytes = J.bits_bytes; T.fuse = J.fuse;
@@ -425,11 +479,13 @@
 		T.ST.image = ctx->s1_image.p; T.ST.heads = ctx->s1_heads.p; T.ST.multi = ctx->s1_multi.p; T.ST.flat = 1;
 	}
 	if(seed2){
-		T.ST2.seeds = st.put(L.s2_seeds.data(), L.s2_seeds.size());
+		const bool resident = seed3 && L.s3_resident;
+		T.ST2.seeds = resident ? nullptr : st.put(L.s2_seeds.data(), L.s2_seeds.size());
 		T.ST2.masks = st.put(reinterpret_cast<const uint4 *>(L.s2_masks.data()), L.s2_masks.size());
 		T.ST2.floors = st.put(L.s2_floors.data(), L.s2_floors.size());
-		T.ST2.n_seeds = (uint32_t)L.s2_seeds.size(); T.ST2.n_or = n_or;
-		if(seed3){ T.d_s3_prefix = st.put(L.s3_prefix.data(), L.s3_prefix.size()); T.d_s3_spans = st.put(L.s3_spans.data(), L.s3_spans.size()); }
+		T.ST2.n_seeds = (uint32_t)P.n_seeds; T.ST2.n_or = n_or;
+		if(resident){ T.d_s3_records = st.put(reinterpret_cast<const uint4 *>(L.s3_records.data()), L.s3_records.size()); T.d_s3_store = ctx->seed_store.base; }
+		else if(seed3){ T.d_s3_prefix = st.put(L.s3_prefix.data(), L.s3_prefix.size()); T.d_s3_spans = st.put(L.s3_spans.data(), L.s3_spans.size()); }
 	}
 	const size_t ctrl_bytes = (8 + 2*(size_t)S.n)*sizeof(uint32_t);
 	if(T.fuse){
@@ -483,10 +539,12 @@
 	return PCR_OK;
 }
 
-void seed3_args(SeqSet &S, const Seed2Tables &Tg, const uint32_t *d_chunk_prefix, const uint8_t *d_spans, const pcr_ctx::S3Launch &L3, const IrrArgs2 &IA, Seed3Tables &T3, Seed3Set &Q3)
+void seed3_args(SeqSet &S, const Seed2Tables &Tg, const uint32_t *d_chunk_prefix, const uint8_t *d_spans, const uint4 *d_records, uint32_t n_rec, const uint32_t *store,
+	const pcr_ctx::S3Launch &L3, const IrrArgs2 &IA, Seed3Tables &T3, Seed3Set &Q3)
 {
 	T3.seeds = Tg.seeds; T3.spans = d_spans; T3.chunk_prefix = d_chunk_prefix; T3.masks = Tg.masks; T3.floors = Tg.floors;
-	T3.n_seeds = Tg.n_seeds; T3.n_or = Tg.n_or; T3.or_base = Tg.or_base;
+	T3.n_seeds = Tg.n_seeds; T3.n_or = Tg.n_or; T3.or_base = Tg.or_base; T3.rec_cap = 0;
+	if(d_records){ T3.records = d_records; T3.store = store; T3.n_rec = n_rec; T3.rec_cap = L3.rec_cap; }
 	T3.pix_first = S.pix_first.p; T3.pix_last = S.pix_last.p; T3.pix_ent = S.pix_ent.p;
 	Q3 = Seed3Set{ S.valid_d(), S.blk_info.p, S.blk_local.p, S.d_active.p };
 	T3.n_chunks = L3.n_chunks; T3.per_wg = L3.per_wg; T3.slice_cap = L3.slice_cap;
@@ -494,14 +552,15 @@
 }
 inline size_t seed3_lds(const Seed3Tables &T3)
 {
+	if(T3.rec_cap) return (size_t)T3.n_or*sizeof(uint4) + 2*(size_t)T3.slice_cap*sizeof(uint32_t) + (((size_t)T3.n_or + 15) & ~size_t(15)) + (((size_t)T3.slice_cap + 1) & ~size_t(1))*sizeof(uint2) + (size_t)T3.rec_cap*sizeof(uint4) + 16;
 	return (size_t)T3.n_or*sizeof(uint4) + 2*(size_t)T3.slice_cap*sizeof(uint32_t) + (((size_t)T3.n_or + 15) & ~size_t(15)) + (((size_t)T3.slice_cap + 15) & ~size_t(15)) + 16;
 }
 
-int launch_seed3_group(pcr_ctx *ctx, SeqSet &S, const Seed2Tables &Tg, const uint32_t *d_chunk_prefix, const uint8_t *d_spans, const pcr_ctx::S3Launch &L3, const IrrArgs2 &IA,
-	const HitSink &sink, const S2Clear &Z)
+int launch_seed3_group(pcr_ctx *ctx, SeqSet &S, const Seed2Tables &Tg, const uint32_t *d_chunk_prefix, const uint8_t *d_spans, const uint4 *d_records, uint32_t n_rec,
+	const uint32_t *store, const pcr_ctx::S3Launch &L3, const IrrArgs2 &IA, const HitSink &sink, const S2Clear &Z)
 {
 	Seed3Tables T3; Seed3Set Q3;
-	seed3_args(S, Tg, d_chunk_prefix, d_spans, L3, IA, T3, Q3);
+	seed3_args(S, Tg, d_chunk_prefix, d_spans, d_records, n_rec, store, L3, IA, T3, Q3);
 	const size_t dyn3 = seed3_lds(T3);
 	if(!ctx->s3_attr_set){
 		HIP_TRY(hipFuncSetAttribute((const void *)k_seed3<S3_WG_THREADS>, hipFuncAttributeMaxDynamicSharedMemorySize, 128*1024));
@@ -553,13 +612,17 @@
 		for(size_t g = 0, b = 0;g < L.s2_group_end.size();++g){ if((size_t)L.s2_group_end[g] - b > (size_t)sgrid.x*S2_THREADS) irr_by_index = false; b = L.s2_group_end[g]; }
 		if(irr_by_index && (rc = irr_index_usable(ctx, S, irr_by_index)) != PCR_OK) return rc;
 	}
-	uint32_t g_begin = 0, g_prefix = 0;
+	const bool resident = seed3 && L.s3_resident;
+	uint32_t g_begin = 0, g_prefix = 0, r_begin = 0;
 	bool first_launch = true;
 	for(size_t g = 0;g < L.s2_group_end.size();++g){
 		Seed2Tables Tg = T.ST2;
 		const uint32_t or0 = L.s2_group_or[g], g_or = L.s2_group_nor[g];
-		const uint8_t *const d_spans = seed3 ? T.d_s3_spans + g_begin : nullptr;
-		Tg.seeds = T.ST2.seeds + g_begin; Tg.n_seeds = L.s2_group_end[g] - g_begin;
+		const uint8_t *const d_spans = (seed3 && !resident) ? T.d_s3_spans + g_begin : nullptr;
+		const uint4 *const d_records = resident ? T.d_s3_records + r_begin : nullptr;
+		const uint32_t n_rec = resident ? L.s3_rec_end[g] - r_begin - 1u : 0u;
+		if(resident) r_begin = L.s3_rec_end[g];
+		Tg.seeds = resident ? nullptr : T.ST2.seeds + g_begin; Tg.n_seeds = L.s2_group_end[g] - g_begin;
 		Tg.masks = T.ST2.masks + (size_t)or0; Tg.floors = T.ST2.floors + or0; Tg.n_or = g_or; Tg.or_base = or0;
 		g_begin = L.s2_group_end[g];
 		if(Tg.n_seeds == 0){ g_prefix += 1u; continue; }
@@ -569,7 +632,7 @@
 			or0, or0 + g_or - 1, g + 1, L.s2_group_end.size(), sizeof(S2Shared), dyn);
 		const S2Clear Z = group_clear(T, fa, sink, first_launch);
 		if(seed3){
-			if((rc = launch_seed3_group(ctx, S, Tg, T.d_s3_prefix + g_prefix, d_spans, L.s3_launch[g], IA, sink, Z)) != PCR_OK) return rc;
+			if((rc = launch_seed3_group(ctx, S, Tg, resident ? nullptr : T.d_s3_prefix + g_prefix, d_spans, d_records, n_rec, T.d_s3_store, L.s3_launch[g], IA, sink, Z)) != PCR_OK) return rc;
 			g_prefix += Tg.n_seeds + 1u;
 		}
 		else hipLaunchKernelGGL(k_seed2_of_ctx, sgrid, sblock, dyn, ctx->stream, S.tb_d(), S.valid_d(), S.tile_desc.p, S.n_tiles, Tg, S.d_active.p, ctx->d_cand_fwd, ctx->d_cand_floor,
@@ -838,6 +901,10 @@
 	uint32_t *const st = J.pair_W.start;
 	for(uint32_t w = 0;w <= Gh;++w) st[w] = L3.W.start[2*w];
 	for(uint32_t w = Gh + 1;w <= S3_MAX_WG/2;++w) st[w] = st[Gh];
+	if(J.L.s3_resident){
+		pcrseed::record_slice_caps(J.L.s3_records.data(), J.L.s3_rec_end[0] - 1u, st, Gh, J.pair_slice_cap, J.pair_rec_cap);
+		return pcrseed::record_lds(J.L.s2_group_nor[0], J.pair_slice_cap, J.pair_rec_cap) <= S3_LDS_BUDGET;
+	}
 	uint32_t cap = 2;
 	for(uint32_t w = 0;w < Gh;++w) cap = std::max(cap, std::min(st[w + 1] + 2u, ns + 1u) - st[w]);
 	J.pair_slice_cap = cap;
@@ -869,7 +936,8 @@
 	Tg.n_seeds = L.s2_group_end[0]; Tg.masks = H.T.ST2.masks + (size_t)L.s2_group_or[0]; Tg.floors = H.T.ST2.floors + L.s2_group_or[0];
 	Tg.n_or = L.s2_group_nor[0]; Tg.or_base = L.s2_group_or[0];
 	H.scan.IA = group_irr_args(S, J.P, L.s2_group_offmask[0], true, J.P.s3_with_irr);
-	seed3_args(S, Tg, H.T.d_s3_prefix, H.T.d_s3_spans, L.s3_launch[0], H.scan.IA, H.scan.T3, H.scan.Q);
+	seed3_args(S, Tg, H.T.d_s3_prefix, H.T.d_s3_spans, H.T.d_s3_records, L.s3_resident ? L.s3_rec_end[0] - 1u : 0u, H.T.d_s3_store, L.s3_launch[0], H.scan.IA, H.scan.T3, H.scan.Q);
+	if(L.s3_resident) H.scan.T3.rec_cap = J.pair_rec_cap;
 	H.scan.T3.per_wg *= 2u; H.scan.T3.slice_cap = J.pair_slice_cap; H.scan.T3.n_irr_wg = (H.scan.T3.n_irr_wg + 1u)/2u;
 	H.scan.cand_fwd = ctx->d_cand_fwd; H.scan.cand_floor = ctx->d_cand_floor; H.scan.sink = H.sink;
 	H.scan.Z = group_clear(H.T, &J.fa, H.sink, true);
diff --git a/profiles/dbg/fresh_oligos.py b/profiles/dbg/fresh_oligos.py
--- /dev/null
+++ b/profiles/dbg/fresh_oligos.py
@@ -0,0 +1,59 @@
+import os
+import sys
+import time
+
+ROOT = os.path.dirname(os.path.dirname(os.path.dirname(os.path.abspath(__file__))))
+sys.path.insert(0, ROOT)
+
+
+def main(n):
+    import numpy as np
+    import torch
+    from pcramp_amd import api, synth, words as W
+
+    thr_t = 1.0
+    thr = float(np.float32(thr_t) * np.float32(0.9))
+    sets = [synth.GlobalSet("C2", 1, seed_base=j) for j in range(3)]
+    pool = [p for gs in sets for p in gs.pairs()]
+    batches = [W.pairs_array([pool[(9 * b + i) % len(pool)] for i in range(50)]) for b in range(16)]
+    st = torch.cuda.Stream()
+    hs = []
+    for gs in sets:
+        s = api.Screener(0, stream=st.cuda_stream)
+        s.load_sequences(*gs.members(0, gs.T))
+        hs.append(s)
+    words = int(hs[0].bitset_words())
+    with torch.cuda.stream(st):
+        out = torch.zeros((3, 2, 50, words), dtype=torch.int64, device="cuda:0")
+    st.synchronize()
+    calls = [[h.screen_call(b, thr, out[j, 0].data_ptr(), out[j, 1].data_ptr(), thr_t, thr_t, 80, 200, False, 18, False, False) for b in batches]
+             for j, h in enumerate(hs)]
+    warm = W.pairs_array(pool[:2])
+    for j, h in enumerate(hs):
+        h.screen_device(warm, thr, out[j, 0].data_ptr(), out[j, 1].data_ptr(), thr_t, thr_t, 80, 200, False)
+    for h in hs:
+        h.synchronize()
+
+    def loop(i0, i1):
+        t0 = time.perf_counter()
+        for i in range(i0, i1):
+            calls[i % 3][(i // 3) % 16]()
+            if i % 48 == 47:
+                for h in hs:
+                    h.synchronize()
+        for h in hs:
+            h.synchronize()
+        st.synchronize()
+        return (time.perf_counter() - t0) * 1e6 / max(1, i1 - i0)
+
+    first = loop(0, 48)
+    rest = loop(48, n)
+    bits = int(np.unpackbits(out.cpu().numpy().view(np.uint8)).sum())
+    for h in hs:
+        h.close()
+    print("fresh_oligos: first round (48 passes, every block new) %.1f us per pass; then %d passes over the 16 batches %.2f us per pass; %d bits set"
+          % (first, n - 48, rest, bits))
+
+
+if __name__ == "__main__":
+    main(int(sys.argv[1]) if len(sys.argv) > 1 else 8048)
```

Result: slower. 26.04 billion (-1.6%).
